# trappmartin/DeepStructuredMixtures

Hardware: AMD Instinct MI355X
Metric: fit!+predict wall-clock, DSMGP N=100k D=8 (lower is better)
Workload: dtype f64

## Files before the change

deepstructuredmixtures_amd/csrc/dsmgp_hip.cpp:

```cpp
#include "../../include/dsmgp_hip.h"
#ifdef DSMGP_DIAG
#include "../../include/dsmgp_hip_diag.h"
#endif
#include "kernels.hpp"
#include "kernels_fused.hpp"

#include <algorithm>
#include <atomic>
#include <cmath>
#include <cstdio>
#include <cstdlib>
#include <cstring>
#include <string>
#include <thread>
#include <array>
#include <chrono>
#include <dlfcn.h>
#include <limits>
#include <vector>

using namespace dsmgp;

namespace {

std::string g_create_error;

struct HyperHost {
    int kind = -1;
    std::vector<double> loghyp;
};

struct LeafHost {
    int n = 0, npad = 0, nb = 0, kid = 0;
    double mean = 0.0;
    int64_t obs_off = 0;
    int op = DSMGP_SHARE_FULL, src = -1;
    int64_t prefix = 0;
    int owner = -1;
    int kb = 0;
    size_t f_off = 0, dinv_off = 0, vec_off = 0, xg_off = 0;
    int nt = 0, ntpad = 0;
    size_t vt_off = 0, xt_off = 0, pv_off = 0;
    int64_t route_off = 0;
};

template <class T>
struct DevBuf {
    T* p = nullptr;
    size_t count = 0;
    size_t cap = 0;

    DevBuf() = default;
    DevBuf(const DevBuf&) = delete;
    DevBuf& operator=(const DevBuf&) = delete;
    DevBuf(DevBuf&& o) noexcept : p(o.p), count(o.count), cap(o.cap) {
        o.p = nullptr;
        o.count = o.cap = 0;
    }
    DevBuf& operator=(DevBuf&& o) noexcept {
        if (this != &o) {
            release();
            std::swap(p, o.p);
            std::swap(count, o.count);
            std::swap(cap, o.cap);
        }
        return *this;
    }
    ~DevBuf() { release(); }

    int grow(dsmgp_ctx* c, size_t need, size_t want);
    int grow(dsmgp_ctx* c, size_t need) { return grow(c, need, std::max<size_t>(1, need + need / 8)); }
    int alloc(dsmgp_ctx* c, size_t n) { return grow(c, n, n); }
    void clear() { count = 0; }
    void release() {
        if (p) (void)hipFree(p);
        p = nullptr;
        count = cap = 0;
    }
    void drop(bool keep) { keep ? clear() : release(); }
};

struct HostLog {
    const char* what;
    std::chrono::steady_clock::time_point t0;
    explicit HostLog(const char* w) : what(w), t0(std::chrono::steady_clock::now()) {}
    void lap(const char* next) {
        done();
        what = next;
        t0 = std::chrono::steady_clock::now();
    }
    void done() {
        static const bool on = std::getenv("DSMGP_HOSTLOG") != nullptr;
        if (on && what)
            std::fprintf(stderr, "hostlog %-28s %.4f s\n", what,
                         std::chrono::duration<double>(std::chrono::steady_clock::now() - t0).count());
        what = nullptr;
    }
    ~HostLog() { done(); }
};

enum { STEP_CLASSIC = 0, STEP_FUSED = 1 };
constexpr int MAX_LANES = 4;
#ifndef DSMGP_FUSED_SHALLOW
#define DSMGP_FUSED_SHALLOW 4
#endif
constexpr int FUSED_SHALLOW_STEPS = DSMGP_FUSED_SHALLOW;
constexpr int FUSED_SHALLOW_MIN_LEAVES = 32;
#ifndef DSMGP_STREAM_FLAGS
#define DSMGP_STREAM_FLAGS hipStreamDefault
#endif
#ifndef DSMGP_LANES_AUTO_MIN
#define DSMGP_LANES_AUTO_MIN 8
#endif
constexpr int LANES_AUTO_MIN_LEAVES = DSMGP_LANES_AUTO_MIN;
#ifndef DSMGP_TAIL_SPLIT_DEFAULT
#define DSMGP_TAIL_SPLIT_DEFAULT 4
#endif
#ifndef DSMGP_TAIL_ROUNDS_DEFAULT
#define DSMGP_TAIL_ROUNDS_DEFAULT 1
#endif
#ifndef DSMGP_TAIL_SPLIT_LANES
#define DSMGP_TAIL_SPLIT_LANES 1
// ... 193 lines not shown
        const size_t T = tiles.size();
        size_t slab = 0;
        if ((int)T < ncu) {
            tail_begin = upd.size();
            emit(tiles, 0, T, choose_split((int)T, K, ncu), slab);
        } else {
            const size_t r = T % (size_t)ncu;
            size_t ntail = r + (T < (size_t)(2 * ncu) ? (size_t)tail_rounds * ncu : 0);
            if (ntail > T) ntail = T;
            int S = std::min(tail_split, std::max(1, K / 256));
            if (r > 0 && r * 4 < (size_t)ncu) S = std::max(S, (int)std::min<size_t>((size_t)ncu / r, 16));
            S = std::min(S, std::max(1, K / 256));
            if (S <= 1 || r == 0) ntail = 0;
            emit(tiles, 0, T - ntail, 1, slab);
            tail_begin = upd.size();
            if (ntail) emit(tiles, T - ntail, T, S, slab);
        }
        max_slabs = std::max(max_slabs, slab);
    }
    int ragged_rounds = 2, ragged_div = 4;
    void add_step_ragged(const std::vector<TileTask>& tiles, int Kavg, int kblocks) {
        const size_t T = tiles.size();
        if (kblocks < 8) {
            add_step(tiles, Kavg);
            return;
        }
        size_t slab = 0;
        size_t cut = 0;
        int maxb;
        if (T < (size_t)((ragged_rounds + 2) * ncu)) {
            long W = 0;
            for (const TileTask& u : tiles) W += (u.k1 - u.k0) / TB;
            maxb = (int)std::min<long>(kblocks, std::max<long>(2, W / (long)(2 * ncu * 3)));
        } else {
            cut = T - (size_t)(ragged_rounds * ncu);
            emit(tiles, 0, cut, 1, slab);
            maxb = std::max(1, kblocks / ragged_div);
        }
        auto pieces = [&](const TileTask& u) { return std::max(1, ((u.k1 - u.k0) / TB + maxb - 1) / maxb); };
        for (size_t i = cut; i < T;) {
            const int S = pieces(tiles[i]);
            size_t j = i + 1;
            while (j < T && pieces(tiles[j]) == S) ++j;
            emit(tiles, i, j, S, slab);
            i = j;
        }
        max_slabs = std::max(max_slabs, slab);
    }
    void bind(double* workspace) {
        for (size_t i = 0; i < upd.size(); ++i)
            if (upd_slab[i] >= 0) upd[i].C = workspace + (size_t)upd_slab[i] * TB * TB;
        for (size_t i = 0; i < red.size(); ++i) red[i].slabs = workspace + (size_t)red_slab[i] * TB * TB;
    }
};

struct SweepLane {
    UpdateSplitter U;
    std::vector<TileTask> trsm;
    std::vector<int> upd_at, red_at, trsm_at;
    void mark(int k) {
        upd_at[(size_t)k] = (int)U.upd.size();
        red_at[(size_t)k] = (int)U.red.size();
        trsm_at[(size_t)k] = (int)trsm.size();
    }
};

}

struct dsmgp_ctx {
    int device = 0;
    hipStream_t stream = nullptr;
    std::string err;
    int profile = 0;
    bool alt_names = false;

    int64_t N = 0;
    int D = 0;
    DevBuf<double> dX, dy;

    int L = 0;
    std::vector<LeafHost> leaves;
    std::vector<int64_t> obs_ptr, obs_idx;
    DevBuf<int64_t> d_obs_ptr, d_obs_idx;
    bool plan_ready = false;

    std::vector<HyperHost> hyper;
    DevBuf<KParam> d_kp;
    DevBuf<double> d_l2;

    double* arenaF = nullptr;
    double* arenaDinv = nullptr;
    double* arenaVec = nullptr;
    double* arenaXg = nullptr;
    DevBuf<int> d_info;
    DevBuf<int> d_owner;
    DevBuf<double> d_mll;
    DevBuf<LeafDev> d_leaves;
    std::vector<LeafDev> h_leaves;
    size_t bytes_needed = 0;

    DevBuf<GramTask> gram;
    bool fuse_gram = true;
    bool fuse_steps = true;
    bool diag_in_update = true;
    std::vector<char> fused_step[2];
    int lanes_opt = 0;
    int nlanes = 1;
    hipStream_t lane_stream[MAX_LANES] = {};
    hipEvent_t ev_fork = nullptr, ev_join[MAX_LANES] = {};
    std::vector<char> leaf_lane;
    StepLists phase[MAX_LANES][2];
    std::vector<char> leaf_group;
    char* pool_base = nullptr;
    size_t pool_cap = 0, pool_top = 0, pool_mark_plan = 0;
    double* slabF[MAX_LANES] = {};
    StepLists phaseJ[MAX_LANES][2];
    double* slabJ[MAX_LANES] = {};
    double alg_flops_joint = 0.0;
    bool joint = true;
    bool joint_ready = false;
    bool vt_valid = false;
    bool last_fit_joint = false;
    int ncu = 256;
    bool xcd_order = true;
    int tail_split = DSMGP_TAIL_SPLIT_DEFAULT, tail_rounds = DSMGP_TAIL_ROUNDS_DEFAULT;
    int tail_split_lanes = DSMGP_TAIL_SPLIT_LANES, tail_rounds_lanes = DSMGP_TAIL_ROUNDS_LANES;
    int ragged_rounds = 2, ragged_div = 4;
    std::vector<int> fwd_off, bwd_off;
    DevBuf<SolveTask> fwd, bwd;
    int solve_steps = 0;
    bool fitted = false;
    bool use_graph = false;
    hipGraphExec_t fit_graph[2] = {nullptr, nullptr};
    int graph_launches[2][2] = {{0, 0}, {0, 0}};
    bool alpha_valid = false;
    bool dinv_complete = false;
    DevBuf<DiagTask> dinvc_prefix;
    DevBuf<DiagTask> dinvc_fwd;
    DevBuf<DiagTask> dinvc_all;

    DevBuf<double> dXt;
    int64_t n_t = 0;
    DevBuf<int64_t> d_route_ptr, d_route_idx;
    std::vector<int64_t> route_ptr;
    double* arenaVt = nullptr;
    size_t arenaVt_count = 0;
    size_t cap_Xt = 0, cap_PV = 0;
    char* stage = nullptr;
    size_t stage_cap = 0, stage_top = 0;
    DevBuf<SweepSeg> psegs;
    double* arenaXt = nullptr;
    double* arenaPV = nullptr;
    size_t acc_off = 0, acc_count = 0;
    DevBuf<PredTask> ptasks_slow;
    DevBuf<GramTask> pgram;
    DevBuf<GramTask> pgram0;
    DevBuf<PredTask> ptasks;
    SweepLists psweep;
    double* arenaCov = nullptr;
    size_t cap_Cov = 0;
    DevBuf<PredCovTask> pcov;
    double* arenaB = nullptr;
    size_t cap_B = 0;
    DevBuf<PredBetaTask> pgbeta;
    DevBuf<PredGradTask> pgtasks;
    DevBuf<PredGradFinTask> pgfin;
    DevBuf<double> d_pgpart;
    DevBuf<double> d_pgout;
    bool test_ready = false;
    bool predicted = false;
    int64_t route_total = 0;

    DevBuf<int64_t> d_row_ptr;
    DevBuf<int32_t> d_row_ent;
    DevBuf<int32_t> d_ent_leaf;
    DevBuf<double> d_agg_part;
    DevBuf<double> d_agg_coef;
    DevBuf<int32_t> d_agg_group;
    DevBuf<double> d_agg_out;
    int agg_family = -1, agg_G = 0, agg_W = 0;
    bool agg_partial_ready = false, agg_done = false;
    bool agg_total = false;

    bool grad_ready = false;
    std::vector<char> grad_active;
    double* arenaX = nullptr;
    size_t arenaX_count = 0;
    DevBuf<TransTask> gtrans;
    SweepLists ginv;
    DevBuf<FrobTask> gfrob;
    std::vector<int> gfrob_leaf;
    DevBuf<GradTask> gdot;
    size_t gdot_prod0 = 0;
    size_t gdot_mat0 = 0;
    std::vector<int> gdot_leaf;
    DevBuf<ArdLinTask> gardlin;
    std::vector<int> gardlin_leaf;
    bool ard_true_gradient = false;
    int gstride = 2;
    std::vector<int> grad_src;
    DevBuf<double> d_gpart;
    size_t gpart_count = 0;
    bool xinv_all = false;
    bool grad_lists_all = false;
    bool grad_all_owners = false;
    std::vector<size_t> gxoff;
    bool loo_ready = false;
    DevBuf<RowNormTask> lrow;
    DevBuf<LooTask> lleaf;
    DevBuf<double> d_loo;
    bool lg_ready = false;
    std::vector<int> lg_kinds;
// ... 211 lines not shown
    }
    S.upd_off[(size_t)nv] = bu;
    S.red_off[(size_t)nv] = br;
    S.trsm_off[(size_t)nv] = bt;
    return 0;
}

void drop_graphs(dsmgp_ctx* c) {
    for (auto& g : c->fit_graph)
        if (g) {
            (void)hipGraphExecDestroy(g);
            g = nullptr;
        }
}

void free_grad_lists(dsmgp_ctx* c) {
    c->gtrans.clear();
    c->ginv.clear();
    c->gfrob.clear();
    c->gdot.clear();
    c->gardlin.clear();
    c->grad_ready = false;
}

void free_grad(dsmgp_ctx* c) {
    c->ginv.release(c);
    arena_put(c, c->arenaX);
    c->gtrans.release();
    c->gfrob.release();
    c->gdot.release();
    c->gardlin.release();
    c->d_gpart.release();
    c->grad_ready = false;
    c->xinv_all = false;
    c->loo_ready = false;
    c->lrow.release();
    c->lleaf.release();
    c->d_loo.release();
    c->lg_ready = false;
    arena_put(c, c->arenaH);
    c->d_lgvec.release();
    c->lgvec.release();
    c->lginv.release();
    c->lghvec.release();
    c->lgdot.release();
    c->lgardlin.release();
    c->d_lgpart.release();
}

void free_tree(dsmgp_ctx* c) {
    c->rtree = RouteTree{};
    c->rt_kind.release();
    c->rt_first.release();
    c->rt_nchild.release();
    c->rt_sdim.release();
    c->rt_leaf.release();
    c->rt_thr.release();
    c->rtree_ready = false;
    c->rtree_nodes = 0;
    c->rtree_max_leaf = -1;
}

void free_test(dsmgp_ctx* c, bool keep = false);
void free_plan(dsmgp_ctx* c) {
    drop_graphs(c);
    if (c->pool_base) {
        free_test(c);
        c->pool_top = 0;
        c->pool_mark_plan = 0;
    }
    arena_put(c, c->arenaF);
    arena_put(c, c->arenaDinv);
    arena_put(c, c->arenaVec);
    arena_put(c, c->arenaXg);
    c->d_info.release();
    c->d_owner.release();
    c->d_mll.release();
    c->d_leaves.release();
    c->gram.release();
    for (auto& lane : c->phase)
        for (auto& ph : lane) ph.drop(false);
    for (auto& sl : c->slabF) arena_put(c, sl);
    c->fwd.release();
    c->bwd.release();
    c->dinvc_prefix.release();
    c->dinvc_fwd.release();
    c->dinvc_all.release();
    free_grad(c);
    c->plan_ready = false;
    c->phase_ready = false;
    c->fitted = false;
}

void free_test(dsmgp_ctx* c, bool keep) {
    drop_graphs(c);
    if (c->pool_base) {
        free_grad(c);
        c->pool_top = c->pool_mark_plan;
        keep = false;
    }
    c->dXt.drop(keep);
    c->d_route_ptr.drop(keep);
    c->d_route_idx.drop(keep);
    c->d_row_ptr.drop(keep);
    c->d_row_ent.drop(keep);
    c->d_ent_leaf.drop(keep);
    c->d_agg_part.drop(keep);
    c->d_agg_coef.drop(keep);
    c->d_agg_group.drop(keep);
    c->d_agg_out.drop(keep);
    c->agg_partial_ready = c->agg_done = c->agg_total = false;
    if (!keep) {
        arena_put(c, c->arenaVt);
        c->arenaVt_count = 0;
        arena_put(c, c->arenaXt);
        arena_put(c, c->arenaPV);
        c->cap_Xt = c->cap_PV = 0;
    }
    c->pgram.drop(keep);
    c->pgram0.drop(keep);
    c->ptasks.drop(keep);
    c->ptasks_slow.drop(keep);
    c->psweep.drop(c, keep);
    c->psegs.drop(keep);
    arena_put(c, c->arenaCov);
    c->cap_Cov = 0;
    c->pcov.drop(keep);
    arena_put(c, c->arenaB);
    c->cap_B = 0;
    c->pgbeta.drop(keep);
    c->pgtasks.drop(keep);
    c->pgfin.drop(keep);
    c->d_pgpart.drop(keep);
    c->d_pgout.drop(keep);
    for (auto& lane : c->phaseJ)
        for (auto& ph : lane) ph.drop(keep);
    for (auto& sl : c->slabJ) arena_put(c, sl);
    c->joint_ready = false;
    c->vt_valid = false;
    c->test_ready = false;
    c->predicted = false;
}

inline int round_up(int x, int m) { return (x + m - 1) / m * m; }
inline int tile_mrows(int valid) {
    const int m = round_up(std::max(0, std::min(TB, valid)), 16);
    return m >= TB ? 0 : std::max(16, m);
}

struct KindInfo {
    const char* name;
    bool ard;
    bool iso_matern;
    bool matern;
    bool linear;
    double nh_num;
    bool per_dim_grad;
    bool contraction;
    bool set_checked;
};
constexpr KindInfo KINDS[] = {
    {"IsoSE",          false, false, false, false, -0.5,  false,  true,  false},
    {"ArdSE",          true,  false, false, false, -0.5,  true,   false, false},
    {"IsoLinear",      false, false, false, true,  -0.5,  false,  false, false},
    {"ArdLinear",      true,  false, false, true,  1.0,   false,  false, false},
    {"ArdSEProduct",   true,  false, false, false, -0.5,  true,   true,  true},
// ... 108 lines not shown

bool gram_fused(const dsmgp_ctx* c) { return c->fuse_gram && c->D <= GRAM_FUSE_MAX_D; }

void push_fused8_tasks(std::vector<FusedTask8>& out, std::vector<RowBlock>& blocks, const LeafDev& d, const LeafHost& lf, int k) {
    for (size_t b0 = 0; b0 < blocks.size(); b0 += 8) {
        FusedTask8 f{};
        f.B = d.F + (size_t)k * TB;
        f.Dinv = d.Dinv + (size_t)k * TB * TB;
        f.gxb = d.Xg + (size_t)k * TB;
        f.ldb = f.gldb = lf.npad;
        f.gnb = std::max(0, std::min(TB, lf.n - k * TB));
        f.k1 = k * TB;
        f.kid = lf.kid;
        f.nblk = (int)std::min<size_t>(8, blocks.size() - b0);
        for (int q = 0; q < f.nblk; ++q) {
            f.rb[q] = blocks[b0 + q];
            if (f.rb[q].wi != nullptr) f.zk = d.z + (size_t)k * TB;
        }
        out.push_back(f);
    }
    blocks.clear();
}

int build_factor_steps(dsmgp_ctx* c, int lane, bool with_test, StepLists (&phase)[2], double*& slab_ws, double& alg_flops,
                       double& alg_flops_fused, bool slab_outside_pool = false) {
    const int L = c->L;
    alg_flops = 0.0;
    const bool fused = gram_fused(c);
    UpdateSplitter split[2] = {make_splitter(c, c->nlanes), make_splitter(c, c->nlanes)};
    for (int ph = 0; ph < 2; ++ph) {
        StepLists& S = phase[ph];
        UpdateSplitter& U = split[ph];
        auto in_phase = [&](const LeafHost& lf) {
            const size_t l = (size_t)(&lf - c->leaves.data());
            return c->leaf_group[l] == ph && c->leaf_lane[l] == lane;
        };
        int nsteps = 0;
        for (int l = 0; l < L; ++l) {
            const LeafHost& lf = c->leaves[l];
            if (!in_phase(lf)) continue;
            if (lf.owner == l || (with_test && lf.nt > 0)) nsteps = std::max(nsteps, lf.nb);
        }
        S.nsteps = nsteps;
        std::vector<TileTask> trsm;
        std::vector<DiagTask> diag;
        std::vector<FusedTask8> ftile8;
        std::vector<RowBlock> blocks8;
        std::vector<DiagFusedTask> fdiag;
        std::vector<DiagFinishTask> dfin;
        S.dpos.assign(nsteps, 0);
        S.dfin_off.assign(nsteps + 1, 0);
        S.upd_off.assign(nsteps + 1, 0);
        S.red_off.assign(nsteps + 1, 0);
        S.trsm_off.assign(nsteps + 1, 0);
        S.diag_off.assign(nsteps + 1, 0);
        S.fdiag_off.assign(nsteps + 1, 0);
        S.ftile8_off.assign(nsteps + 1, 0);
        S.step_tiles.assign(nsteps, 0);
        S.pad.assign(nsteps, 0);
        S.mode.assign(nsteps, STEP_CLASSIC);
        for (int k = 0; k < nsteps; ++k) {
            S.upd_off[k] = (int)U.upd.size();
            S.red_off[k] = (int)U.red.size();
            S.trsm_off[k] = (int)trsm.size();
            S.diag_off[k] = (int)diag.size();
            S.fdiag_off[k] = (int)fdiag.size();
            S.ftile8_off[k] = (int)ftile8.size();
            S.dfin_off[k] = (int)dfin.size();
            const int mode = k < (int)c->fused_step[ph].size() ? c->fused_step[ph][k] : STEP_CLASSIC;
            S.mode[k] = (char)mode;
            const bool fstep = mode != STEP_CLASSIC;
            std::vector<TileTask> tiles;
            auto classic_at = [&](int q) {
                return q >= 0 && q < nsteps && (q >= (int)c->fused_step[ph].size() || c->fused_step[ph][q] == STEP_CLASSIC);
            };
            const bool finish_here = c->diag_in_update && gram_fused(c) && !fstep && k >= 2 && classic_at(k - 1);
            const bool ahead = c->diag_in_update && gram_fused(c) && !fstep && k >= 1 && classic_at(k + 1);
            size_t nsym = 0;
            for (int l = 0; l < L; ++l) {
                const LeafHost& lf = c->leaves[l];
                if (lf.nb <= k || !in_phase(lf)) continue;
                const LeafDev& d = c->h_leaves[l];
                const int ld = lf.npad;
                if (lf.owner == l) {
                    const int i_first = (k < lf.kb) ? lf.kb : k;
                    const bool own_diag = (k >= lf.kb);
                    const bool fin = finish_here && own_diag;
                    for (int i = i_first; i < lf.nb; ++i) {
                        if (fstep) {
                            if (i == k) continue;
                            const int rows = std::max(0, std::min(TB, lf.n - i * TB));
                            for (int r = 0; r < rows; r += 16) {
                                RowBlock b{};
                                b.A = d.F + (size_t)i * TB + r;
                                b.C = d.F + (size_t)i * TB + r + (size_t)k * TB * ld;
                                b.gx = d.Xg + (size_t)i * TB + r;
                                b.lda = b.ldc = b.glda = ld;
                                b.nvalid = std::min(16, rows - r);
                                if (ph != 1) b.wi = d.w + (size_t)i * TB + r;
                                blocks8.push_back(b);
                            }
                            continue;
                        }
                        if (k > 0 && !(i == k && fin)) {
                            TileTask u{};
                            u.A = d.F + (size_t)i * TB;
                            u.B = d.F + (size_t)k * TB;
                            u.C = d.F + (size_t)i * TB + (size_t)k * TB * ld;
                            u.lda = u.ldb = u.ldc = ld;
                            u.k0 = 0;
                            u.k1 = k * TB;
                            u.update = 1;
                            u.mrows = tile_mrows(lf.n - i * TB);
                            u.sym = (i == k) ? 1 : 0;
                            nsym += (size_t)u.sym;
                            if (fused) {
                                u.gram = 1 | (i == k ? 2 : 0) | 4;
                                u.kid = lf.kid;
                                u.gxa = d.Xg + (size_t)i * TB;
                                u.gxb = d.Xg + (size_t)k * TB;
                                u.glda = u.gldb = ld;
                                u.gna = std::max(0, std::min(TB, lf.n - i * TB));
                                u.gnb = std::max(0, std::min(TB, lf.n - k * TB));
                            }
                            tiles.push_back(u);
                        }
                        if (i == k + 1 && ahead && k + 1 >= lf.kb) {
                            TileTask u{};
                            u.A = u.B = d.F + (size_t)i * TB;
                            u.C = d.F + (size_t)i * TB + (size_t)i * TB * ld;
                            u.lda = u.ldb = u.ldc = ld;
                            u.k0 = 0;
                            u.k1 = k * TB;
                            u.update = 1;
                            u.mrows = tile_mrows(lf.n - i * TB);
                            u.sym = 1;
                            nsym += 1;
                            u.gram = 1 | 2 | 4;
                            u.kid = lf.kid;
                            u.gxa = u.gxb = d.Xg + (size_t)i * TB;
                            u.glda = u.gldb = ld;
                            u.gna = u.gnb = std::max(0, std::min(TB, lf.n - i * TB));
                            tiles.push_back(u);
                        }
                        if (i > k) {
                            TileTask s{};
                            s.A = d.F + (size_t)i * TB + (size_t)k * TB * ld;
                            s.B = d.Dinv + (size_t)k * TB * TB;
                            s.C = const_cast<double*>(s.A);
                            s.lda = ld;
                            s.ldb = TB;
                            s.ldc = ld;
                            s.k0 = 0;
                            s.k1 = TB;
                            s.update = 0;
                            s.mrows = tile_mrows(lf.n - i * TB);
                            if (ph != 1) {
                                s.zk = d.z + (size_t)k * TB;
                                s.wi = d.w + (size_t)i * TB;
                            }
                            trsm.push_back(s);
                        }
                    }
                    if (own_diag) {
                        DiagTask g{};
                        g.T = d.F + (size_t)k * TB + (size_t)k * TB * ld;
                        g.Dinv = d.Dinv + (size_t)k * TB * TB;
                        if (ph != 1) {
                            g.wk = d.w + (size_t)k * TB;
                            g.zk = d.z + (size_t)k * TB;
                        }
                        g.info = d.info;
                        g.ld = ld;
                        g.nvalid = std::max(0, std::min(TB, lf.n - k * TB));
                        g.row0 = k * TB;
                        if (fstep) {
                            DiagFusedTask fg{};
                            fg.d = g;
                            fg.A = d.F + (size_t)k * TB;
                            fg.gx = d.Xg + (size_t)k * TB;
                            fg.k1 = k * TB;
                            fg.glda = ld;
                            fg.kid = lf.kid;
                            fdiag.push_back(fg);
                        } else if (fin) {
                            DiagFinishTask ft{};
                            ft.d = g;
                            ft.A = d.F + (size_t)k * TB + (size_t)(k - 1) * TB * ld;
                            dfin.push_back(ft);
                        } else {
                            diag.push_back(g);
                        }
                    }
                }
                if (with_test && lf.nt > 0) {
                    for (int ti = 0; ti < lf.ntpad / TB; ++ti) {
                        double* tile = d.Vt + (size_t)ti * TB + (size_t)k * TB * lf.ntpad;
                        if (fstep) {
                            const int rows = std::max(0, std::min(TB, lf.nt - ti * TB));
                            for (int r = 0; r < rows; r += 16) {
                                RowBlock b{};
                                b.A = d.Vt + (size_t)ti * TB + r;
                                b.C = tile + r;
                                b.gx = d.Xtg + (size_t)ti * TB + r;
                                b.lda = b.ldc = b.glda = lf.ntpad;
                                b.nvalid = std::min(16, rows - r);
                                if (d.zfused) {
                                    b.wi = d.macc + (size_t)ti * TB + r;
                                    b.sq = d.sacc + (size_t)ti * TB + r;
                                }
                                blocks8.push_back(b);
                            }
                            continue;
                        }
                        if (k > 0) {
                            TileTask u{};
                            u.A = d.Vt + (size_t)ti * TB;
                            u.B = d.F + (size_t)k * TB;
                            u.C = tile;
                            u.lda = lf.ntpad;
                            u.ldb = ld;
                            u.ldc = lf.ntpad;
                            u.k0 = 0;
                            u.k1 = k * TB;
                            u.update = 1;
                            u.mrows = tile_mrows(lf.nt - ti * TB);
                            if (fused) {
                                u.gram = 1;
                                u.kid = lf.kid;
                                u.gxa = d.Xtg + (size_t)ti * TB;
                                u.gxb = d.Xg + (size_t)k * TB;
                                u.glda = lf.ntpad;
                                u.gldb = ld;
                                u.gna = std::max(0, std::min(TB, lf.nt - ti * TB));
                                u.gnb = std::max(0, std::min(TB, lf.n - k * TB));
                            }
                            tiles.push_back(u);
                        }
                        TileTask s{};
                        s.A = tile;
                        s.B = d.Dinv + (size_t)k * TB * TB;
                        s.C = tile;
                        s.lda = lf.ntpad;
                        s.ldb = TB;
                        s.ldc = lf.ntpad;
                        s.k0 = 0;
                        s.k1 = TB;
                        s.update = 0;
                        s.mrows = tile_mrows(lf.nt - ti * TB);
                        if (d.zfused) {
                            s.zk = d.z + (size_t)k * TB;
// ... 153 lines not shown
        HIPCHK(c, hipMemcpy(c->d_owner.p, owner.data(), (size_t)L * sizeof(int), hipMemcpyHostToDevice));
    }
    if (int rc = c->d_mll.alloc(c, L)) return rc;
    if (int rc = c->d_leaves.alloc(c, L)) return rc;

    c->h_leaves.assign(L, LeafDev{});
    for (int l = 0; l < L; ++l) {
        const LeafHost& lf = c->leaves[l];
        LeafDev& d = c->h_leaves[l];
        d.F = c->arenaF + lf.f_off;
        d.Dinv = c->arenaDinv + lf.dinv_off;
        d.Xg = c->arenaXg + lf.xg_off;
        d.yc = c->arenaVec + lf.vec_off;
        d.w = d.yc + lf.npad;
        d.z = d.w + lf.npad;
        d.alpha = d.z + lf.npad;
        d.info = c->d_info.p + lf.owner;
        d.mean = lf.mean;
        d.n = lf.n;
        d.npad = lf.npad;
        d.nb = lf.nb;
        d.kid = lf.kid;
    }
    HIPCHK(c, hipMemcpy(c->d_leaves.p, c->h_leaves.data(), L * sizeof(LeafDev), hipMemcpyHostToDevice));

    {
        int maxpad = 0;
        for (auto& lf : c->leaves) maxpad = std::max(maxpad, lf.npad);
        for (int l0 = 0; l0 < L; l0 += 32768) {
            const int cnt = std::min(32768, L - l0);
            dim3 grid((maxpad + 255) / 256, cnt);
            gather_leaf_kernel<<<grid, 256, 0, c->stream>>>(c->d_leaves.p, c->d_obs_ptr.p, c->d_obs_idx.p, c->dX.p, c->dy.p,
                                                            c->N, c->D, l0);
        }
        HIPCHK(c, hipGetLastError());
    }
    std::vector<ZeroRowsTask> zr;
    if (gram_fused(c)) {
        for (int l = 0; l < L; ++l) {
            const LeafHost& lf = c->leaves[l];
            const int last = lf.n - (lf.nb - 1) * TB;
            if (lf.owner != l || lf.nb < 2 || last >= TB) continue;
            ZeroRowsTask z{};
            z.p = c->h_leaves[l].F + (size_t)(lf.nb - 1) * TB;
            z.ld = lf.npad;
            z.r0 = (std::max(0, last) + 15) / 16 * 16;
            z.ncols = (lf.nb - 1) * TB;
            if (z.r0 < TB) zr.push_back(z);
        }
    }
    std::vector<ZeroUpperTask> zu;
    int maxnb = 1;
    for (int l = 0; l < L; ++l) {
        const LeafHost& lf = c->leaves[l];
        if (lf.owner != l) continue;
        zu.push_back(ZeroUpperTask{c->h_leaves[l].F, lf.npad, lf.nb});
        maxnb = std::max(maxnb, lf.nb);
    }
    {
        DevBuf<ZeroRowsTask> zrows;
        DevBuf<ZeroUpperTask> zupper;
        if (int rc = dev_upload(c, zrows, zr)) return rc;
        if (int rc = dev_upload(c, zupper, zu)) return rc;
        if (!zr.empty()) zero_pad_rows_kernel<<<(int)zr.size(), 256, 0, c->stream>>>(zrows.p);
        for (size_t b0 = 0; b0 < zu.size(); b0 += 32768) {
            const size_t cnt = std::min<size_t>(32768, zu.size() - b0);
            zero_upper_blocks_kernel<<<dim3((unsigned)cnt, (unsigned)std::min(maxnb, 64)), 256, 0, c->stream>>>(zupper.p + b0);
        }
        const hipError_t e1 = hipGetLastError(), e2 = hipStreamSynchronize(c->stream);
        HIPCHK(c, e1);
        HIPCHK(c, e2);
    }

    c->leaf_group.assign(L, 0);
    for (int l = 0; l < L; ++l)
        if (c->leaves[l].op == DSMGP_SHARE_PREFIX) c->leaf_group[l] = 1;
    {
        std::vector<int> unit(L);
        std::vector<double> cost(L, 0.0);
        for (int l = 0; l < L; ++l) {
            const LeafHost& lf = c->leaves[l];
            unit[l] = lf.op == DSMGP_SHARE_FULL ? l : lf.src;
            const double n = (double)lf.n;
            cost[unit[l]] += lf.op == DSMGP_SHARE_COPY ? n * n : n * n * n;
        }
        int nunits = 0;
        for (int l = 0; l < L; ++l) nunits += unit[l] == l ? 1 : 0;
        c->nlanes = c->lanes_opt > 0 ? c->lanes_opt : (nunits >= LANES_AUTO_MIN_LEAVES ? 2 : 1);
        c->nlanes = std::max(1, std::min(c->nlanes, nunits));
        c->leaf_lane.assign(L, 0);
        if (c->nlanes > 1) {
            std::vector<int> order;
            for (int l = 0; l < L; ++l)
                if (unit[l] == l) order.push_back(l);
            std::stable_sort(order.begin(), order.end(), [&](int a, int b) { return cost[a] > cost[b]; });
            double load[MAX_LANES] = {};
            std::vector<char> of_unit(L, 0);
            for (int u : order) {
                int lane = 0;
                for (int q = 1; q < c->nlanes; ++q)
                    if (load[q] < load[lane]) lane = q;
                of_unit[u] = (char)lane;
                load[lane] += cost[u];
            }
            for (int l = 0; l < L; ++l) c->leaf_lane[l] = of_unit[unit[l]];
        }
    }
    for (int ph = 0; ph < 2; ++ph) {
        int ns = 0;
        for (int l = 0; l < L; ++l)
            if (c->leaf_group[l] == ph) ns = std::max(ns, c->leaves[l].nb);
        c->fused_step[ph].assign(ns, STEP_CLASSIC);
        if (!gram_fused(c)) continue;
        for (int k = 0; k < ns; ++k) {
            int nd = 0;
            for (int l = 0; l < L; ++l) {
                const LeafHost& lf = c->leaves[l];
                if (c->leaf_group[l] == ph && lf.owner == l && lf.nb > k && k >= lf.kb) ++nd;
            }
            if (c->fuse_steps && (nd > c->ncu || (k <= FUSED_SHALLOW_STEPS && nd >= FUSED_SHALLOW_MIN_LEAVES))) c->fused_step[ph][k] = STEP_FUSED;
        }
    }
    std::vector<GramTask> gram;
    const bool fused = gram_fused(c);
    for (int l = 0; l < L; ++l) {
        const LeafHost& lf = c->leaves[l];
        if (lf.owner != l) continue;
        {
            const std::vector<char>& fs = c->fused_step[(int)c->leaf_group[l]];
            if (fused && !fs.empty() && fs[0] != STEP_CLASSIC) continue;
        }
        const LeafDev& d = c->h_leaves[l];
        for (int j = 0; j < (fused ? 1 : lf.nb); ++j)
            for (int i = (fused ? std::max(j, lf.kb) : j); i < lf.nb; ++i) {
                GramTask g{};
                g.xa = d.Xg + (size_t)i * TB;
                g.xb = d.Xg + (size_t)j * TB;
                g.out = d.F + (size_t)i * TB + (size_t)j * TB * lf.npad;
                g.lda = g.ldb = g.ldo = lf.npad;
                g.na = std::max(0, std::min(TB, lf.n - i * TB));
                g.nb = std::max(0, std::min(TB, lf.n - j * TB));
                g.sym = 1;
                g.diag = (i == j);
                g.kid = lf.kid;
                gram.push_back(g);
            }
    }
    if (int rc = dev_upload(c, c->gram, gram)) return rc;

    {
        auto fused_in = [&](int ph, int k) { return k < (int)c->fused_step[ph].size() && c->fused_step[ph][k] == STEP_FUSED; };
        auto block_task = [&](int l, int k) {
            const LeafHost& lf = c->leaves[l];
            const LeafDev& d = c->h_leaves[l];
            DiagTask g{};
            g.T = d.F + (size_t)k * TB + (size_t)k * TB * lf.npad;
            g.Dinv = d.Dinv + (size_t)k * TB * TB;
            g.info = d.info;
            g.ld = lf.npad;
            g.nvalid = std::max(0, std::min(TB, lf.n - k * TB));
            g.row0 = k * TB;
            return g;
        };
        std::vector<DiagTask> pre, fw;
        std::vector<char> done(L, 0);
        for (int l = 0; l < L; ++l) {
            const LeafHost& lf = c->leaves[l];
            if (lf.op == DSMGP_SHARE_PREFIX)
                for (int k = 0; k < lf.kb; ++k)
                    if (fused_in(0, k)) pre.push_back(block_task(l, k));
            if (lf.op == DSMGP_SHARE_FULL) continue;
            const int o = lf.owner;
            if (done[o]) continue;
            done[o] = 1;
            const LeafHost& lo = c->leaves[o];
            const int pho = (int)c->leaf_group[o];
            for (int k = lo.kb; k < lo.nb; ++k)
                if (fused_in(pho, k)) fw.push_back(block_task(o, k));
        }
        if (int rc = dev_upload(c, c->dinvc_prefix, pre)) return rc;
        if (int rc = dev_upload(c, c->dinvc_fwd, fw)) return rc;
        std::vector<DiagTask> all;
        for (int l = 0; l < L; ++l) {
            const LeafHost& lf = c->leaves[l];
            if (lf.owner != l) continue;
            for (int k = lf.kb; k < lf.nb; ++k)
                if (fused_in((int)c->leaf_group[l], k)) all.push_back(block_task(l, k));
        }
        if (int rc = dev_upload(c, c->dinvc_all, all)) return rc;
    }
    c->phase_ready = false;

    {
        int nsteps = 0;
        for (auto& lf : c->leaves) nsteps = std::max(nsteps, lf.nb);
        c->solve_steps = nsteps;
        std::vector<SolveTask> fwd, bwd;
        c->fwd_off.assign(nsteps + 1, 0);
        c->bwd_off.assign(nsteps + 1, 0);
        for (int k = 0; k < nsteps; ++k) {
            c->fwd_off[k] = (int)fwd.size();
            for (int l = 0; l < L; ++l) {
                const LeafHost& lf = c->leaves[l];
                if (lf.nb <= k) continue;
                if (lf.owner == l && lf.op == DSMGP_SHARE_FULL) continue;
                const LeafDev& d = c->h_leaves[l];
                for (int i = k; i < lf.nb; ++i) {
                    SolveTask s{};
                    s.Dk = d.Dinv + (size_t)k * TB * TB;
                    s.vk = d.w + (size_t)k * TB;
                    s.ldt = lf.npad;
                    if (i == k) {
                        s.self = 1;
                        s.out_k = d.z + (size_t)k * TB;
                    } else {
                        s.T = d.F + (size_t)i * TB + (size_t)k * TB * lf.npad;
                        s.vi = d.w + (size_t)i * TB;
                    }
                    fwd.push_back(s);
                }
            }
        }
        c->fwd_off[nsteps] = (int)fwd.size();
        for (int s_ = 0; s_ < nsteps; ++s_) {
            c->bwd_off[s_] = (int)bwd.size();
            for (int l = 0; l < L; ++l) {
                const LeafHost& lf = c->leaves[l];
                const LeafDev& d = c->h_leaves[l];
                if (s_ == 0) {
                    SolveTask s{};
                    s.self = 1;
                    s.Dk = d.Dinv + (size_t)(lf.nb - 1) * TB * TB;
                    s.vk = d.w + (size_t)(lf.nb - 1) * TB;
                    s.out_k = d.alpha + (size_t)(lf.nb - 1) * TB;
                    s.ldt = lf.npad;
                    bwd.push_back(s);
                    continue;
                }
                const int kb = lf.nb - s_;
                if (kb < 1) continue;
                for (int j = 0; j < kb; ++j) {
                    SolveTask s{};
                    s.T = d.F + (size_t)kb * TB + (size_t)j * TB * lf.npad;
                    s.ldt = lf.npad;
                    s.vk = d.alpha + (size_t)kb * TB;
                    s.vi = d.w + (size_t)j * TB;
                    if (j == kb - 1) {
                        s.Dk = d.Dinv + (size_t)j * TB * TB;
                        s.out_k = d.alpha + (size_t)j * TB;
                    }
                    bwd.push_back(s);
                }
            }
        }
        c->bwd_off[nsteps] = (int)bwd.size();
        if (int rc = dev_upload(c, c->fwd, fwd)) return rc;
        if (int rc = dev_upload(c, c->bwd, bwd)) return rc;
    }
    HIPCHK(c, hipStreamSynchronize(c->stream));
    c->plan_ready = true;
    c->pool_mark_plan = c->pool_top;
    return 0;
}

int ensure_phase(dsmgp_ctx* c) {
    if (c->phase_ready) return 0;
    HostLog hl("ensure_phase: factor steps");
    c->alg_flops_update = c->alg_flops_fused = 0.0;
    for (int lane = 0; lane < c->nlanes; ++lane) {
        double fu = 0.0, ff = 0.0;
        if (int rc = build_factor_steps(c, lane, false, c->phase[lane], c->slabF[lane], fu, ff, true)) return rc;
        c->alg_flops_update += fu;
        c->alg_flops_fused += ff;
    }
    HIPCHK(c, hipStreamSynchronize(c->stream));
    c->phase_ready = true;
    return 0;
}

int ensure_joint(dsmgp_ctx* c) {
    if (c->joint_ready) return 0;
    HostLog hl("ensure_joint: joint factor steps");
    c->alg_flops_joint = c->alg_flops_fused_joint = 0.0;
    for (int lane = 0; lane < c->nlanes; ++lane) {
        double fu = 0.0, ff = 0.0;
        if (int rc = build_factor_steps(c, lane, true, c->phaseJ[lane], c->slabJ[lane], fu, ff)) return rc;
        c->alg_flops_joint += fu;
        c->alg_flops_fused_joint += ff;
    }
    HIPCHK(c, hipStreamSynchronize(c->stream));
    c->joint_ready = true;
    return 0;
}

void launch_tiles(dsmgp_ctx* c, const TileTask* tasks, int n, int role = 0 , bool pad = false,
                  int dpos = 0, const DiagFinishTask* dfin = nullptr, int ndfin = 0, hipStream_t st = nullptr) {
    const int g = n + ndfin;
    if (!st) st = c->stream;
    if (pad) {
        if (role == 1) tile_trsm_kernel<true><<<n, 256, 0, st>>>(tasks);
        else if (c->profile == 0 || c->alt_names) tile_gemm_kernel_v2<false, 2, true><<<g, 256, 0, st>>>(tasks, nullptr, c->d_kp.p, c->D, dpos, dfin, ndfin);
        else tile_gemm_kernel_v2<false, 0, true><<<g, 256, 0, st>>>(tasks, nullptr, c->d_kp.p, c->D, dpos, dfin, ndfin);
        return;
    }
    if (role == 1) tile_trsm_kernel<false><<<n, 256, 0, st>>>(tasks);
    else if (c->profile == 0 || c->alt_names) tile_gemm_kernel_v2<false, 2><<<g, 256, 0, st>>>(tasks, nullptr, c->d_kp.p, c->D, dpos, dfin, ndfin);
// ... 114 lines not shown
        pt.end(st);
        const int nr = S.red_off[k + 1] - S.red_off[k];
        if (nr > 0) {
            pt.begin(13, st);
            tile_reduce_kernel<<<nr * REDUCE_WGS, 256, 0, st>>>(S.red.p + S.red_off[k]);
            pt.end(st);
        }
        if (count_launches) c->n_update_launches++;
    }
    const int nd = S.diag_off[k + 1] - S.diag_off[k];
    if (nd > 0) {
        pt.begin(2, st);
        chol_diag_packed_kernel<<<nd, 256, DIAGP_LDS_BYTES, st>>>(S.diag.p + S.diag_off[k]);
        pt.note(k, nd, 0);
        pt.end(st);
    }
    const int ns = S.trsm_off[k + 1] - S.trsm_off[k];
    if (ns > 0) {
        pt.begin(3, st);
        launch_tiles(c, S.trsm.p + S.trsm_off[k], ns, 1, S.pad[k] != 0, 0, nullptr, 0, st);
        pt.note(k, ns, 0);
        pt.end(st);
    }
}

int fork_lanes(dsmgp_ctx* c, int nl) {
    if (nl > 1) {
        HIPCHK(c, hipEventRecord(c->ev_fork, c->stream));
        for (int lane = 1; lane < nl; ++lane) HIPCHK(c, hipStreamWaitEvent(c->lane_stream[lane], c->ev_fork, 0));
    }
    return 0;
}
int join_lanes(dsmgp_ctx* c, int nl) {
    for (int lane = 1; lane < nl; ++lane) {
        HIPCHK(c, hipEventRecord(c->ev_join[lane], c->lane_stream[lane]));
        HIPCHK(c, hipStreamWaitEvent(c->stream, c->ev_join[lane], 0));
    }
    return 0;
}

int run_lanes(dsmgp_ctx* c, StepLists (*lists)[2], int ph, PhaseTimer& pt, bool count_launches) {
    int nsteps = 0;
    for (int lane = 0; lane < c->nlanes; ++lane) nsteps = std::max(nsteps, lists[lane][ph].nsteps);
    if (nsteps == 0) return 0;
    if (int rc = fork_lanes(c, c->nlanes)) return rc;
    for (int k = 0; k < nsteps; ++k)
        for (int lane = 0; lane < c->nlanes; ++lane) run_step(c, lists[lane][ph], k, pt, c->lane_stream[lane], count_launches);
    HIPCHK(c, hipGetLastError());
    return join_lanes(c, c->nlanes);
}

int ensure_dinv(dsmgp_ctx* c) {
    if (c->dinv_complete) return 0;
    if (c->dinvc_all.count)
        dinv_complete_kernel<<<(int)c->dinvc_all.count, 256, DIAGP_LDS_BYTES, c->stream>>>(c->dinvc_all.p);
    HIPCHK(c, hipGetLastError());
    c->dinv_complete = true;
    return 0;
}

int ensure_alpha(dsmgp_ctx* c) {
    if (c->alpha_valid) return 0;
    if (int rc = ensure_dinv(c)) return rc;
    EventPair ev;
    HIPCHK(c, ev.init());
    HIPCHK(c, hipEventRecord(ev.a, c->stream));
    int maxpad = 0;
    for (auto& lf : c->leaves) maxpad = std::max(maxpad, lf.npad);
    copy_z_kernel<<<dim3((maxpad + 255) / 256, c->L), 256, 0, c->stream>>>(c->d_leaves.p);
    for (int s = 0; s < c->solve_steps; ++s) {
        const int n = c->bwd_off[s + 1] - c->bwd_off[s];
        if (n > 0) solve_bwd_kernel<<<n, 256, 0, c->stream>>>(c->bwd.p + c->bwd_off[s]);
    }
    HIPCHK(c, hipGetLastError());
    HIPCHK(c, hipEventRecord(ev.b, c->stream));
    HIPCHK(c, hipStreamSynchronize(c->stream));
    float ms = 0.f;
    HIPCHK(c, hipEventElapsedTime(&ms, ev.a, ev.b));
    c->timings[14] = ms * 1e-3;
    c->alpha_valid = true;
    return 0;
}

}

extern "C" {

int dsmgp_create(int32_t device_id, dsmgp_ctx** out) {
    if (!out) return fail(nullptr, DSMGP_E_ARG, "out is NULL");
    *out = nullptr;
    int ndev = 0;
    if (hipGetDeviceCount(&ndev) != hipSuccess || ndev == 0)
        return fail(nullptr, DSMGP_E_NODEVICE, "no HIP device visible: the GP-expert path has no CPU fallback");
    if (device_id < 0 || device_id >= ndev) return fail(nullptr, DSMGP_E_ARG, "device id out of range");
    dsmgp_ctx* c = new dsmgp_ctx();
    c->device = device_id;
    if (hipSetDevice(device_id) != hipSuccess || hipStreamCreateWithFlags(&c->stream, DSMGP_STREAM_FLAGS) != hipSuccess) {
        delete c;
        return fail(nullptr, DSMGP_E_HIP, "cannot initialise device");
    }
    c->lane_stream[0] = c->stream;
    bool lanes_ok = hipEventCreateWithFlags(&c->ev_fork, hipEventDisableTiming) == hipSuccess;
    for (int lane = 1; lane < MAX_LANES && lanes_ok; ++lane)
        lanes_ok = hipStreamCreateWithFlags(&c->lane_stream[lane], DSMGP_STREAM_FLAGS) == hipSuccess &&
                   hipEventCreateWithFlags(&c->ev_join[lane], hipEventDisableTiming) == hipSuccess;
    if (!lanes_ok) {
        (void)hipStreamDestroy(c->stream);
        delete c;
        return fail(nullptr, DSMGP_E_HIP, "cannot create the lanes' streams");
    }
    (void)hipFuncSetAttribute(reinterpret_cast<const void*>(chol_diag_packed_kernel),
                              hipFuncAttributeMaxDynamicSharedMemorySize, DIAGP_LDS_BYTES);
    (void)hipFuncSetAttribute(reinterpret_cast<const void*>(dinv_complete_kernel),
                              hipFuncAttributeMaxDynamicSharedMemorySize, DIAGP_LDS_BYTES);
    {
        hipDeviceProp_t prop;
        if (hipGetDeviceProperties(&prop, device_id) == hipSuccess && prop.multiProcessorCount > 0)
            c->ncu = prop.multiProcessorCount;
    }
#ifdef DSMGP_DIAG
    if (const char* s = std::getenv("DSMGP_XCD")) c->xcd_order = std::atoi(s) != 0;
    if (const char* s = std::getenv("DSMGP_TAIL_SPLIT")) c->tail_split = c->tail_split_lanes = std::max(1, std::atoi(s));
    if (const char* s = std::getenv("DSMGP_TAIL_ROUNDS")) c->tail_rounds = c->tail_rounds_lanes = std::max(0, std::atoi(s));
    if (const char* s = std::getenv("DSMGP_RAGGED_ROUNDS")) c->ragged_rounds = std::max(1, std::atoi(s));
    if (const char* s = std::getenv("DSMGP_RAGGED_DIV")) c->ragged_div = std::max(1, std::atoi(s));
#endif
    const char* p = std::getenv("DSMGP_PROFILE");
    c->profile = p ? std::atoi(p) * 2 : 0;
    *out = c;
    return 0;
}

int dsmgp_destroy(dsmgp_ctx* c) {
    if (!c) return DSMGP_E_ARG;
    (void)hipSetDevice(c->device);
    free_plan(c);
    free_test(c);
    if (c->pool_base) (void)hipFree(c->pool_base);
    c->pool_base = nullptr;
    (void)dsmgp_comm_destroy(c);
    drop_graphs(c);
    if (c->side) {
        (void)hipStreamSynchronize(c->side);
        (void)hipStreamDestroy(c->side);
    }
    if (c->stage) (void)hipHostFree(c->stage);
    c->stage = nullptr;
    for (hipEvent_t e : c->event_pool) (void)hipEventDestroy(e);
    if (c->ev_fork) (void)hipEventDestroy(c->ev_fork);
    for (int lane = 1; lane < MAX_LANES; ++lane) {
        if (c->ev_join[lane]) (void)hipEventDestroy(c->ev_join[lane]);
        if (c->lane_stream[lane]) (void)hipStreamDestroy(c->lane_stream[lane]);
    }
    if (c->stream) (void)hipStreamDestroy(c->stream);
    delete c;
    return 0;
}

const char* dsmgp_last_error(dsmgp_ctx* c) { return c ? c->err.c_str() : g_create_error.c_str(); }

int dsmgp_device_name(dsmgp_ctx* c, char* buf, int32_t len) {
    if (!c || !buf || len <= 0) return DSMGP_E_ARG;
    hipDeviceProp_t prop;
    HIPCHK(c, hipGetDeviceProperties(&prop, c->device));
    std::snprintf(buf, len, "%s (%s, %d CUs)", prop.name, prop.gcnArchName, prop.multiProcessorCount);
    return 0;
}

int dsmgp_set_joint(dsmgp_ctx* c, int32_t on) {
    if (!c) return DSMGP_E_ARG;
    c->joint = on != 0;
    return 0;
}

int dsmgp_set_option(dsmgp_ctx* c, int32_t option, int32_t value) {
    if (!c) return DSMGP_E_ARG;
    if (option == DSMGP_OPT_ARD_LENGTHSCALE_GRADIENT) {
        if ((value != 0) != c->ard_true_gradient) {
            HIPCHK(c, hipSetDevice(c->device));
            free_grad(c);
        }
        c->ard_true_gradient = value != 0;
        return 0;
    }
    if (option == DSMGP_OPT_FUSED_GRAM) {
        if ((value != 0) != c->fuse_gram) {
            HIPCHK(c, hipSetDevice(c->device));
            free_plan(c);
            free_test(c);
        }
        c->fuse_gram = value != 0;
        return 0;
    }
    if (option == DSMGP_OPT_FUSED_STEPS) {
        if ((value != 0) != c->fuse_steps) {
            HIPCHK(c, hipSetDevice(c->device));
            free_plan(c);
            free_test(c);
        }
        c->fuse_steps = value != 0;
        return 0;
    }
    if (option == DSMGP_OPT_FIT_GRAPH) {
        if (value == 0) drop_graphs(c);
        c->use_graph = value != 0;
        return 0;
    }
    if (option == DSMGP_OPT_LANES) {
        if (value < 0 || value > MAX_LANES) return fail(c, DSMGP_E_ARG, "set_option: lanes must be 0 (automatic) or 1 .. 4");
        if (value != c->lanes_opt) {
            HIPCHK(c, hipSetDevice(c->device));
            free_plan(c);
            free_test(c);
        }
        c->lanes_opt = value;
        return 0;
    }
    if (option == DSMGP_OPT_DIAG_IN_UPDATE) {
        if ((value != 0) != c->diag_in_update) {
            HIPCHK(c, hipSetDevice(c->device));
            free_plan(c);
            free_test(c);
        }
        c->diag_in_update = value != 0;
        return 0;
    }
    return fail(c, DSMGP_E_ARG, "set_option: unknown option");
}

int dsmgp_set_profile(dsmgp_ctx* c, int32_t on) {
    if (!c) return DSMGP_E_ARG;
    c->alt_names = on == 3;
    c->profile = on < 0 ? 0 : (on == 3 ? 1 : (on > 2 ? 2 : on));
    return 0;
}

int dsmgp_set_train(dsmgp_ctx* c, const double* X, const double* y, int64_t N, int32_t D) {
    if (!c) return DSMGP_E_ARG;
    if (!X || !y || N <= 0 || D <= 0) return fail(c, DSMGP_E_ARG, "set_train: bad arguments");
    HIPCHK(c, hipSetDevice(c->device));
    free_plan(c);
    free_test(c);
    free_tree(c);
    c->dX.release();
    c->dy.release();
    c->N = N;
    c->D = D;
    if (int rc = c->dX.alloc(c, (size_t)N * D)) return rc;
    if (int rc = c->dy.alloc(c, (size_t)N)) return rc;
    HIPCHK(c, hipMemcpy(c->dX.p, X, (size_t)N * D * sizeof(double), hipMemcpyHostToDevice));
    HIPCHK(c, hipMemcpy(c->dy.p, y, (size_t)N * sizeof(double), hipMemcpyHostToDevice));
    c->L = 0;
    c->leaves.clear();
    return 0;
}

int dsmgp_set_leaves(dsmgp_ctx* c, int32_t L, const int64_t* obs_ptr, const int64_t* obs_idx,
                     const int32_t* kernel_id, const double* mean) {
    if (!c) return DSMGP_E_ARG;
    if (!c->dX.p) return fail(c, DSMGP_E_STATE, "set_leaves before set_train");
    if (L <= 0 || !obs_ptr || !obs_idx || !kernel_id || !mean) return fail(c, DSMGP_E_ARG, "set_leaves: bad arguments");
    HIPCHK(c, hipSetDevice(c->device));
    free_plan(c);
    free_test(c);
    free_tree(c);
    if (obs_ptr[0] != 0) return fail(c, DSMGP_E_ARG, "obs_ptr[0] must be 0");
    c->leaves.assign(L, LeafHost{});
    c->grad_active.clear();
    for (int l = 0; l < L; ++l) {
        const int64_t a = obs_ptr[l], b = obs_ptr[l + 1];
        if (b <= a) return fail(c, DSMGP_E_ARG, "leaf " + std::to_string(l) + " has no observations");
        if (b - a > (int64_t)1 << 20) return fail(c, DSMGP_E_ARG, "leaf too large");
        for (int64_t i = a; i < b; ++i) {
            if (obs_idx[i] < 0 || obs_idx[i] >= c->N) return fail(c, DSMGP_E_ARG, "observation index out of range");
            if (i > a && obs_idx[i] <= obs_idx[i - 1]) return fail(c, DSMGP_E_ARG, "obs lists must be strictly ascending");
        }
        if (kernel_id[l] < 0 || kernel_id[l] >= DSMGP_MAX_KERNEL_IDS) return fail(c, DSMGP_E_ARG, "kernel id out of range");
        LeafHost& lf = c->leaves[l];
        lf.n = (int)(b - a);
        lf.npad = round_up(lf.n, TB);
        lf.nb = lf.npad / TB;
        lf.kid = kernel_id[l];
        lf.mean = mean[l];
        lf.obs_off = a;
    }
    c->L = L;
    c->obs_ptr.assign(obs_ptr, obs_ptr + L + 1);
    c->obs_idx.assign(obs_idx, obs_idx + obs_ptr[L]);
    c->d_obs_ptr.release();
    c->d_obs_idx.release();
    if (int rc = c->d_obs_ptr.alloc(c, (size_t)L + 1)) return rc;
    if (int rc = c->d_obs_idx.grow(c, c->obs_idx.size(), std::max<size_t>(1, c->obs_idx.size()))) return rc;
    HIPCHK(c, hipMemcpy(c->d_obs_ptr.p, obs_ptr, (L + 1) * sizeof(int64_t), hipMemcpyHostToDevice));
    HIPCHK(c, hipMemcpy(c->d_obs_idx.p, obs_idx, c->obs_idx.size() * sizeof(int64_t), hipMemcpyHostToDevice));
    return 0;
}

int dsmgp_set_sharing(dsmgp_ctx* c, const int32_t* op, const int32_t* src, const int64_t* prefix_len) {
    if (!c) return DSMGP_E_ARG;
    if (c->L == 0) return fail(c, DSMGP_E_STATE, "set_sharing before set_leaves");
    const int L = c->L;
    struct Share { int op; int src; int64_t prefix; };
    std::vector<Share> sh(L, Share{DSMGP_SHARE_FULL, -1, 0});
    for (int l = 0; l < L; ++l) {
        const LeafHost& lf = c->leaves[l];
        const int o = op ? op[l] : DSMGP_SHARE_FULL;
        if (o == DSMGP_SHARE_FULL) continue;
        if (!src || src[l] < 0 || src[l] >= L || src[l] == l) return fail(c, DSMGP_E_ARG, "sharing: bad source leaf");
        const LeafHost& s = c->leaves[src[l]];
        const int so = op[src[l]];
        if (so != DSMGP_SHARE_FULL) return fail(c, DSMGP_E_ARG, "sharing: source leaf must be factorised in full");
        if (s.kid != lf.kid) return fail(c, DSMGP_E_ARG, "sharing: kernel ids differ");
        const int64_t* a = c->obs_idx.data() + lf.obs_off;
        const int64_t* b = c->obs_idx.data() + s.obs_off;
        if (o == DSMGP_SHARE_COPY) {
            if (s.n != lf.n || std::memcmp(a, b, sizeof(int64_t) * lf.n) != 0)
                return fail(c, DSMGP_E_ARG, "sharing: COPY needs identical observation lists");
            sh[l] = Share{o, src[l], 0};
        } else if (o == DSMGP_SHARE_PREFIX) {
            if (!prefix_len || prefix_len[l] != s.n || s.n >= lf.n || std::memcmp(a, b, sizeof(int64_t) * s.n) != 0)
                return fail(c, DSMGP_E_ARG, "sharing: PREFIX needs the source's list as a strict prefix");
            sh[l] = Share{o, src[l], prefix_len[l]};
        } else {
            return fail(c, DSMGP_E_ARG, "sharing: unknown op");
        }
    }
    HIPCHK(c, hipSetDevice(c->device));
    free_plan(c);
    free_test(c);
    for (int l = 0; l < L; ++l) {
        c->leaves[l].op = sh[l].op;
        c->leaves[l].src = sh[l].src;
        c->leaves[l].prefix = sh[l].prefix;
    }
    return 0;
}

int dsmgp_set_hyper(dsmgp_ctx* c, int32_t kernel_id, int32_t kind, const double* loghyp, int32_t n) {
    if (!c) return DSMGP_E_ARG;
    if (kernel_id < 0 || kernel_id >= DSMGP_MAX_KERNEL_IDS || !loghyp || n < 3) return fail(c, DSMGP_E_ARG, "set_hyper: bad arguments");
    if (kind < 0 || kind > DSMGP_KIND_ARD_MATERN52) return fail(c, DSMGP_E_ARG, "set_hyper: unknown kernel kind");
    const KindInfo& ki = KINDS[kind];
    if (ki.set_checked && ki.ard && c->D > 0 && n != c->D + 2)
        return fail(c, DSMGP_E_ARG, std::string("set_hyper: ") + ki.name + " needs one lengthscale per input dimension");
    if (ki.set_checked && !ki.ard && n != 3)
        return fail(c, DSMGP_E_ARG, std::string("set_hyper: ") + ki.name + " takes [logl, logs, logNoise]");
    for (int i = 0; i < n; ++i)
        if (!std::isfinite(loghyp[i])) return fail(c, DSMGP_E_ARG, "set_hyper: non-finite hyper-parameter");
    if ((int)c->hyper.size() <= kernel_id) c->hyper.resize(kernel_id + 1);
    const bool had_matern = any_matern(c);
    if (c->hyper[kernel_id].kind != kind) free_grad(c);
    c->hyper[kernel_id].kind = kind;
    c->hyper[kernel_id].loghyp.assign(loghyp, loghyp + n);
    if (any_matern(c) != had_matern) drop_graphs(c);
    c->fitted = false;
    c->predicted = false;
    c->vt_valid = false;
    return 0;
}

int dsmgp_fit(dsmgp_ctx* c, double* mll_out, int32_t* info_out, double* seconds) {
    if (!c) return DSMGP_E_ARG;
    if (c->L == 0) return fail(c, DSMGP_E_STATE, "fit before set_leaves");
    HIPCHK(c, hipSetDevice(c->device));
    if (int rc = check_hyper(c)) return rc;
    if (!c->plan_ready)
        if (int rc = build_plan(c)) return rc;
    if (int rc = upload_hyper(c)) return rc;
    const bool joint = c->joint && c->test_ready;
    if (joint) {
        if (int rc = ensure_joint(c)) return rc;
    } else if (int rc = ensure_phase(c)) {
        return rc;
    }
    const int L = c->L;
    for (int i = 0; i < 6; ++i) c->timings[i] = 0.0;
    c->timings[11] = 0.0;
    c->timings[13] = 0.0;
    c->timings[14] = 0.0;
    c->timings[18] = c->timings[19] = c->timings[20] = 0.0;
    c->n_update_launches = 0;
    c->n_fused_launches = 0;
    PhaseTimer pt(c);
    EventPair ev;
    HIPCHK(c, ev.init());
    const hipEvent_t t0 = ev.a, t1 = ev.b;
    HIPCHK(c, hipEventRecord(t0, c->stream));

    StepLists (*phases)[2] = joint ? c->phaseJ : c->phase;
    auto enqueue = [&]() -> int {
        HIPCHK(c, hipMemsetAsync(c->d_info.p, 0, L * sizeof(int), c->stream));
        if (joint && c->acc_count) HIPCHK(c, hipMemsetAsync(c->arenaPV + c->acc_off, 0, c->acc_count * sizeof(double), c->stream));
        {
            const DevBuf<GramTask>& tg = (joint && gram_fused(c)) ? c->pgram0 : c->pgram;
            pt.begin(0);
            if (c->gram.count) gram_tile_kernel<<<2 * (int)c->gram.count, 256, 0, c->stream>>>(c->gram.p, c->d_kp.p, c->D);
            if (joint && tg.count) gram_tile_kernel<<<2 * (int)tg.count, 256, 0, c->stream>>>(tg.p, c->d_kp.p, c->D);
            pt.end();
        }
        {
            int maxpad = 0;
            for (auto& lf : c->leaves) maxpad = std::max(maxpad, lf.npad);
            copy_vec_kernel<<<dim3((maxpad + 255) / 256, L), 256, 0, c->stream>>>(c->d_leaves.p);
        }
        if (int rc = run_lanes(c, phases, 0, pt, true)) return rc;
        bool any_prefix = false;
        for (int l = 0; l < L; ++l) {
            const LeafHost& lf = c->leaves[l];
            if (lf.op != DSMGP_SHARE_PREFIX) continue;
            any_prefix = true;
            const LeafDev& d = c->h_leaves[l];
            const LeafDev& s = c->h_leaves[lf.src];
            const size_t rows = (size_t)lf.kb * TB;
            HIPCHK(c, hipMemcpy2DAsync(d.F, (size_t)d.npad * sizeof(double), s.F, (size_t)s.npad * sizeof(double),
                                       rows * sizeof(double), rows, hipMemcpyDeviceToDevice, c->stream));
            HIPCHK(c, hipMemcpyAsync(d.Dinv, s.Dinv, rows * TB * sizeof(double), hipMemcpyDeviceToDevice, c->stream));
        }
        if (any_prefix) {
            if (c->dinvc_prefix.count)
                dinv_complete_kernel<<<(int)c->dinvc_prefix.count, 256, DIAGP_LDS_BYTES, c->stream>>>(c->dinvc_prefix.p);
            if (int rc = run_lanes(c, phases, 1, pt, true)) return rc;
        }
        {
            pt.begin(4);
            if (c->dinvc_fwd.count)
                dinv_complete_kernel<<<(int)c->dinvc_fwd.count, 256, DIAGP_LDS_BYTES, c->stream>>>(c->dinvc_fwd.p);
            for (int k = 0; k < c->solve_steps; ++k) {
                const int n = c->fwd_off[k + 1] - c->fwd_off[k];
                if (n > 0) solve_fwd_kernel<<<n, 256, 0, c->stream>>>(c->fwd.p + c->fwd_off[k]);
            }
            pt.end();
        }
        pt.begin(5);
        mll_kernel<<<L, 256, 0, c->stream>>>(c->d_leaves.p, c->d_mll.p);
        pt.end();
        return 0;
    };
    c->vt_valid = false;
    c->alpha_valid = false;
    c->xinv_all = false;
    const int gk = joint ? 1 : 0;
    if (c->use_graph && c->profile == 0) {
        if (!c->fit_graph[gk]) {
            hipGraph_t g = nullptr;
            HIPCHK(c, hipStreamBeginCapture(c->stream, hipStreamCaptureModeThreadLocal));
            const int rc = enqueue();
            const hipError_t ce = hipStreamEndCapture(c->stream, &g);
            if (rc != 0 || ce != hipSuccess || !g) {
                if (g) (void)hipGraphDestroy(g);
                (void)hipGetLastError();
                c->use_graph = false;
                if (rc != 0) return rc;
            } else {
                const hipError_t ie = hipGraphInstantiate(&c->fit_graph[gk], g, nullptr, nullptr, 0);
                (void)hipGraphDestroy(g);
                if (ie != hipSuccess) {
                    c->fit_graph[gk] = nullptr;
                    (void)hipGetLastError();
                    c->use_graph = false;
                }
                c->graph_launches[gk][0] = c->n_update_launches;
                c->graph_launches[gk][1] = c->n_fused_launches;
            }
        }
        if (c->fit_graph[gk]) {
            HIPCHK(c, hipGraphLaunch(c->fit_graph[gk], c->stream));
            c->n_update_launches = c->graph_launches[gk][0];
            c->n_fused_launches = c->graph_launches[gk][1];
        } else if (int rc = enqueue()) {
            return rc;
        }
    } else {
        if (int rc = enqueue()) return rc;
    }
    HIPCHK(c, hipGetLastError());
    HIPCHK(c, hipEventRecord(t1, c->stream));
    HIPCHK(c, hipStreamSynchronize(c->stream));
    float ms = 0.f;
    HIPCHK(c, hipEventElapsedTime(&ms, t0, t1));
    pt.collect(t0);
    c->timings[11] = ms * 1e-3;
    if (seconds) *seconds = ms * 1e-3;
    if (mll_out) HIPCHK(c, hipMemcpy(mll_out, c->d_mll.p, L * sizeof(double), hipMemcpyDeviceToHost));
    if (info_out) {
        std::vector<int> owner_info(L);
        HIPCHK(c, hipMemcpy(owner_info.data(), c->d_info.p, L * sizeof(int), hipMemcpyDeviceToHost));
        for (int l = 0; l < L; ++l) info_out[l] = owner_info[c->leaves[l].owner];
    }
    c->fitted = true;
    c->predicted = false;
    c->vt_valid = joint;
    c->last_fit_joint = joint;
    c->dinv_complete = c->dinvc_all.count == 0;
    return 0;
}

}

namespace {
int register_test(dsmgp_ctx* c, HostLog& hl) {
    const int L = c->L;
    const int64_t n_t = c->n_t, total = c->route_total;
    const int64_t* rp = c->route_ptr.data();
    hl.lap("set_test: sizes");
    size_t vTot = 0, xTot = 0;
    size_t accTot = 0;
    for (int l = 0; l < L; ++l) accTot += (size_t)round_up((int)(rp[l + 1] - rp[l]), TB);
    const size_t pTot = 2 * (size_t)total + 2 * accTot + 2 * TB;
    for (int l = 0; l < L; ++l) {
        LeafHost& lf = c->leaves[l];
        lf.nt = (int)(rp[l + 1] - rp[l]);
        lf.ntpad = round_up(lf.nt, TB);
        lf.route_off = rp[l];
        lf.vt_off = vTot;
        vTot += (size_t)lf.ntpad * lf.npad;
        lf.xt_off = xTot;
        xTot += (size_t)lf.ntpad * c->D;
        lf.pv_off = (size_t)rp[l];
    }
    size_t freeB = 0, totalB = 0;
    HIPCHK(c, hipMemGetInfo(&freeB, &totalB));
    const size_t need = (vTot + xTot + pTot) * sizeof(double) + (size_t)n_t * c->D * sizeof(double);
    if (!c->pool_base) freeB += (c->arenaVt_count + c->cap_Xt + c->cap_PV) * sizeof(double);
    if (!c->pool_base && need + (size_t(1) << 30) > freeB)
        return fail(c, DSMGP_E_NOMEM, "test set needs " + std::to_string(need >> 20) + " MiB, device has " +
                                          std::to_string(freeB >> 20) + " MiB free");
    hl.lap("set_test: arenas");
    auto arena_fit = [&](double*& p, size_t& cap, size_t need_) -> int {
        if (c->pool_base) return arena_get(c, p, need_);
        if (p && cap >= need_ && cap <= 2 * need_ + (size_t(1) << 20)) return 0;
        arena_put(c, p);
        cap = 0;
        const size_t want = need_ + need_ / 8;
        if (int rc = arena_get(c, p, want)) return rc;
        cap = want;
        return 0;
    };
    if (int rc = arena_fit(c->arenaVt, c->arenaVt_count, vTot)) return rc;
    if (int rc = arena_fit(c->arenaXt, c->cap_Xt, xTot)) return rc;
    if (int rc = arena_fit(c->arenaPV, c->cap_PV, pTot)) return rc;
    int maxpad = 0;
    size_t accOff = 0;
    c->acc_off = 2 * (size_t)total;
    c->acc_count = 2 * accTot;
    for (int l = 0; l < L; ++l) {
        const LeafHost& lf = c->leaves[l];
        LeafDev& d = c->h_leaves[l];
        d.Vt = c->arenaVt + lf.vt_off;
        d.Xtg = c->arenaXt + lf.xt_off;
        d.mu = c->arenaPV + lf.pv_off;
        d.var = c->arenaPV + (size_t)total + lf.pv_off;
        d.macc = c->arenaPV + 2 * (size_t)total + accOff;
        d.sacc = d.macc + accTot;
        d.zfused = (lf.owner == l && lf.op == DSMGP_SHARE_FULL) ? 1 : 0;
        accOff += (size_t)lf.ntpad;
        d.nt = lf.nt;
        d.ntpad = lf.ntpad;
        maxpad = std::max(maxpad, lf.ntpad);
    }
    if (int rc = stage_upload(c, c->d_leaves.p, c->h_leaves.data(), (size_t)L * sizeof(LeafDev))) return rc;
    if (maxpad > 0) {
        for (int l0 = 0; l0 < L; l0 += 32768) {
            const int cnt = std::min(32768, L - l0);
            gather_test_kernel<<<dim3((maxpad + 255) / 256, cnt), 256, 0, c->stream>>>(
                c->d_leaves.p, c->d_route_ptr.p, c->d_route_idx.p, c->dXt.p, n_t, c->D, l0);
        }
        HIPCHK(c, hipGetLastError());
    }
    hl.lap("set_test: task lists (host)");
    auto fused_at = [&](int l, int k) {
        const std::vector<char>& fs = c->fused_step[(int)c->leaf_group[l]];
        return gram_fused(c) && k < (int)fs.size() && fs[(size_t)k] == STEP_FUSED;
    };
    std::vector<GramTask> pg, pg0;
    std::vector<PredTask> ptk, ptk_slow;
    int nsteps = 0;
    for (int l = 0; l < L; ++l) {
        const LeafHost& lf = c->leaves[l];
        if (lf.nt == 0) continue;
        nsteps = std::max(nsteps, lf.nb);
        const LeafDev& d = c->h_leaves[l];
        for (int ti = 0; ti < lf.ntpad / TB; ++ti) {
            ptk.push_back(PredTask{l, ti * TB});
            if (!d.zfused) ptk_slow.push_back(PredTask{l, ti * TB});
            for (int j = 0; j < lf.nb; ++j) {
                if (fused_at(l, j)) continue;
                if (j > 0 && gram_fused(c)) continue;
                GramTask g{};
                g.xa = d.Xtg + (size_t)ti * TB;
                g.xb = d.Xg + (size_t)j * TB;
                g.out = d.Vt + (size_t)ti * TB + (size_t)j * TB * lf.ntpad;
                g.lda = lf.ntpad;
                g.ldb = lf.npad;
                g.ldo = lf.ntpad;
                g.na = std::max(0, std::min(TB, lf.nt - ti * TB));
                g.nb = std::max(0, std::min(TB, lf.n - j * TB));
                g.sym = 0;
                g.diag = 0;
                g.kid = lf.kid;
                pg.push_back(g);
                if (j == 0) pg0.push_back(g);
            }
        }
    }
    const int nl = c->nlanes, nv = nl * nsteps;
    std::vector<SweepLane> lanes = sweep_lanes(c, nl, nsteps);
    std::vector<int>& f8_off = c->psweep.f8_off;
    f8_off.assign((size_t)nv + 1, 0);
    std::vector<SweepSeg> segs;
    std::vector<std::vector<int>> classic((size_t)nv);
    {
        std::vector<int> cnt8((size_t)nv, 0);
        for (int l = 0; l < L; ++l) {
            const LeafHost& lf = c->leaves[l];
            if (lf.nt == 0) continue;
            const int nt8 = ((lf.nt + 15) / 16 + 7) / 8;
            const size_t v0 = (size_t)c->leaf_lane[l] * (size_t)nsteps;
            for (int k = 0; k < lf.nb; ++k) {
                if (fused_at(l, k)) cnt8[v0 + (size_t)k] += nt8;
                else classic[v0 + (size_t)k].push_back(l);
            }
        }
        for (int v = 0; v < nv; ++v) f8_off[(size_t)v + 1] = f8_off[(size_t)v] + cnt8[(size_t)v];
        std::vector<int> cursor((size_t)nv, 0);
        segs.reserve((size_t)L * 4);
        for (int l = 0; l < L; ++l) {
            const LeafHost& lf = c->leaves[l];
            if (lf.nt == 0) continue;
            const int nt8 = ((lf.nt + 15) / 16 + 7) / 8;
            const size_t v0 = (size_t)c->leaf_lane[l] * (size_t)nsteps;
            for (int k = 0; k < lf.nb; ++k)
                if (fused_at(l, k)) {
                    SweepSeg sg{};
                    sg.leaf = l;
                    sg.k = k;
                    sg.src0 = cursor[v0 + (size_t)k];
                    sg.begin = f8_off[v0 + (size_t)k];
// ... 961 lines not shown
        c->grad_all_owners = false;
        if (rc) return rc;
    }
    return 0;
}
int xinv_fill(dsmgp_ctx* c) {
    if (c->xinv_all) return 0;
    if (c->gtrans.count) transpose_tile_kernel<<<(int)c->gtrans.count * 16, 256, 0, c->stream>>>(c->gtrans.p);
    return run_sweep(c, c->ginv, nullptr);
}

int build_loo_plan(dsmgp_ctx* c) {
    const int L = c->L;
    std::vector<size_t> poff(L, 0);
    size_t pTot = 0;
    for (int l = 0; l < L; ++l) {
        const LeafHost& lf = c->leaves[l];
        if (lf.owner != l) continue;
        poff[l] = pTot;
        pTot += (size_t)lf.npad * ((lf.n + ROWNORM_COLS - 1) / ROWNORM_COLS);
    }
    const size_t nobs = (size_t)c->obs_ptr[L];
    if (int rc = c->d_loo.alloc(c, pTot + 2 * nobs + (size_t)L)) return rc;
    std::vector<RowNormTask> rows;
    std::vector<LooTask> lt((size_t)L);
    for (int l = 0; l < L; ++l) {
        const LeafHost& lf = c->leaves[l];
        const LeafHost& ow = c->leaves[lf.owner];
        lt[l].P = c->d_loo.p + poff[lf.owner];
        lt[l].alpha = c->h_leaves[c->grad_src[l] >= 0 ? c->grad_src[l] : l].alpha;
        lt[l].off = (long long)c->obs_ptr[l];
        lt[l].ldp = ow.npad;
        if (lf.owner != l) continue;
        for (int t = 0; t * TB < lf.n; ++t)
            for (int c0 = t * TB, k = 0; c0 < lf.n; c0 += ROWNORM_COLS, ++k) {
                RowNormTask r{};
                r.X = c->arenaX + c->gxoff[l] + (size_t)t * TB;
                r.out = c->d_loo.p + poff[l] + (size_t)k * lf.npad + (size_t)t * TB;
                r.ld = lf.npad;
                r.col0 = c0;
                r.col1 = std::min(c0 + ROWNORM_COLS, lf.n);
                r.nrows = std::min(TB, lf.n - t * TB);
                rows.push_back(r);
            }
    }
    if (int rc = dev_upload(c, c->lrow, rows)) return rc;
    if (int rc = dev_upload(c, c->lleaf, lt)) return rc;
    c->loo_ready = true;
    return 0;
}
}

int dsmgp_loo(dsmgp_ctx* c, double* mu_out, double* var_out, double* lpd_out, double* seconds) {
    if (!c) return DSMGP_E_ARG;
    if (seconds) *seconds = 0.0;
    if (!c->fitted) return fail(c, DSMGP_E_STATE, "loo before fit");
    HIPCHK(c, hipSetDevice(c->device));
    const int L = c->L;
    OwnGradLists own_lists{c};
    if (int rc = xinv_lists(c, own_lists)) return rc;
    if (!c->loo_ready)
        if (int rc = build_loo_plan(c)) return rc;
    EventPair ev;
    HIPCHK(c, ev.init());
    HIPCHK(c, hipEventRecord(ev.a, c->stream));
    if (int rc = ensure_dinv(c)) return rc;
    if (int rc = ensure_alpha(c)) return rc;
    if (int rc = xinv_fill(c)) return rc;
    const size_t nobs = (size_t)c->obs_ptr[L];
    double* dmu = c->d_loo.p + (c->d_loo.count - 2 * nobs - (size_t)L);
    double* dvar = dmu + nobs;
    double* dlpd = dvar + nobs;
    if (c->lrow.count) rownorm_kernel<<<(unsigned)c->lrow.count, 256, 0, c->stream>>>(c->lrow.p);
    loo_moments_kernel<<<L, 256, 0, c->stream>>>(c->d_leaves.p, c->lleaf.p, c->d_obs_idx.p, c->dy.p, dmu, dvar, dlpd);
    HIPCHK(c, hipGetLastError());
    HIPCHK(c, hipEventRecord(ev.b, c->stream));
    HIPCHK(c, hipStreamSynchronize(c->stream));
    c->xinv_all = true;
    float ms = 0.f;
    HIPCHK(c, hipEventElapsedTime(&ms, ev.a, ev.b));
    if (seconds) *seconds = ms * 1e-3;
    if (mu_out) HIPCHK(c, hipMemcpy(mu_out, dmu, nobs * sizeof(double), hipMemcpyDeviceToHost));
    if (var_out) HIPCHK(c, hipMemcpy(var_out, dvar, nobs * sizeof(double), hipMemcpyDeviceToHost));
    if (lpd_out) HIPCHK(c, hipMemcpy(lpd_out, dlpd, (size_t)L * sizeof(double), hipMemcpyDeviceToHost));
    return 0;
}

int dsmgp_predict_gradients(dsmgp_ctx* c, double* dmu_out, double* dvar_out, int64_t ld, double* seconds) {
    if (!c) return DSMGP_E_ARG;
    if (seconds) *seconds = 0.0;
    if (!c->predicted || !c->vt_valid) return fail(c, DSMGP_E_STATE, "predict_gradients before predict_run on the current fit");
    const size_t nr = (size_t)c->route_total;
    if (nr == 0) return 0;
    if (ld < c->route_total) return fail(c, DSMGP_E_ARG, "predict_gradients: ld < route_total");
    HIPCHK(c, hipSetDevice(c->device));
    const int L = c->L, D = c->D;
    const bool var = dvar_out != nullptr;
    OwnGradLists own_lists{c};
    std::vector<size_t> boff((size_t)L, 0);
    if (var) {
        if (int rc = xinv_lists(c, own_lists)) return rc;
        size_t bTot = 0;
        for (int l = 0; l < L; ++l) {
            const LeafHost& lf = c->leaves[l];
            if (lf.nt == 0) continue;
            boff[l] = bTot;
            bTot += (size_t)lf.ntpad * lf.npad;
        }
        if (int rc = slab_grow(c, c->arenaB, c->cap_B, bTot)) return rc;
    }
    const size_t planes = (var ? 2 : 1) * (size_t)D * TB;
    std::vector<PredBetaTask> beta;
    std::vector<PredGradTask> tasks;
    std::vector<PredGradFinTask> fin;
    for (int l = 0; l < L; ++l) {
        const LeafHost& lf = c->leaves[l];
        if (lf.nt == 0) continue;
        const int nslab = (lf.n + PGRAD_SLAB - 1) / PGRAD_SLAB;
        for (int i = 0; i < lf.ntpad / TB; ++i) {
            PredGradFinTask f{};
            f.nslab = nslab;
            f.nrows = std::min(TB, lf.nt - i * TB);
            fin.push_back(f);
            for (int s = 0; s < nslab; ++s) tasks.push_back(PredGradTask{});
        }
    }
    if (int rc = c->d_pgpart.grow(c, tasks.size() * planes)) return rc;
    if (int rc = c->d_pgout.grow(c, (var ? 2 : 1) * nr * (size_t)D)) return rc;
    size_t ti = 0, fi = 0;
    for (int l = 0; l < L; ++l) {
        const LeafHost& lf = c->leaves[l];
        if (lf.nt == 0) continue;
        const LeafDev& d = c->h_leaves[l];
        const int nslab = (lf.n + PGRAD_SLAB - 1) / PGRAD_SLAB;
        double* Bl = var ? c->arenaB + boff[l] : nullptr;
        for (int i = 0; i < lf.ntpad / TB; ++i) {
            PredGradFinTask& f = fin[fi++];
            f.part = c->d_pgpart.p + ti * planes;
            f.xt = d.Xtg + (size_t)i * TB;
            f.dmu = c->d_pgout.p + (size_t)lf.route_off + (size_t)i * TB;
            f.dvar = var ? f.dmu + nr * (size_t)D : nullptr;
            f.info = d.info;
            f.pstride = (long long)planes;
            f.ldo = (long long)nr;
            f.ldt = lf.ntpad;
            f.kid = lf.kid;
            for (int s = 0; s < nslab; ++s) {
                PredGradTask& g = tasks[ti];
                g.xt = f.xt;
                g.xg = d.Xg;
                g.alpha = d.alpha;
                g.B = var ? Bl + (size_t)i * TB : nullptr;
                g.part = c->d_pgpart.p + ti * planes;
                g.ldt = lf.ntpad;
                g.ldg = lf.npad;
                g.nrows = f.nrows;
                g.c0 = s * PGRAD_SLAB;
                g.c1 = std::min(lf.n, g.c0 + PGRAD_SLAB);
                g.kid = lf.kid;
                ++ti;
            }
            if (!var) continue;
            const LeafHost& ow = c->leaves[lf.owner];
            for (int j = 0; j * TB < lf.n; ++j) {
                PredBetaTask b{};
                b.gemm.A = d.Vt + (size_t)i * TB;
// ... 304 lines not shown
        } else if (h.kind == DSMGP_KIND_ISO_LINEAR) {
            g[0] = -2.0 * (trMKy - cc * trM);
            g[1] = 0.0;
        } else if (h.kind == DSMGP_KIND_ARD_LINEAR) {
            for (int d = 0; d < nl; ++d)
                g[d] = -2.0 * (U[s * D + d] * A[s * D + d] - Q[s * D + d]) / std::exp(2.0 * h.loghyp[d]);
            g[nl] = 0.0;
        } else {
            if (KINDS[h.kind].iso_matern) {
                double sl = 0.0;
                for (int d = 0; d < D; ++d) sl += Sd[s * D + d];
                g[0] = sl;
            } else {
                for (int d = 0; d < nl; ++d) g[d] = Sd[s * D + d];
            }
            g[nl] = 2.0 * SK[s];
        }
        g[nl + 1] = 2.0 * noise * trM;
    }
    if (lpd_out) std::memcpy(lpd_out, lpd.data(), (size_t)L * sizeof(double));
    return 0;
}

int dsmgp_kernel_matrix(dsmgp_ctx* c, int32_t kernel_id, const double* x1, int64_t n1, const double* x2,
                        int64_t n2, double* K_out) {
    if (!c) return DSMGP_E_ARG;
    if (!x1 || !x2 || !K_out || n1 <= 0 || n2 <= 0 || c->D <= 0) return fail(c, DSMGP_E_ARG, "kernel_matrix: bad arguments");
    if (kernel_id < 0 || kernel_id >= (int)c->hyper.size() || c->hyper[kernel_id].kind < 0)
        return fail(c, DSMGP_E_STATE, "kernel_matrix: kernel id without hyper-parameters");
    if (ard_linear_short(c, kernel_id))
        return fail(c, DSMGP_E_ARG, std::string("kernel_matrix: ") + KINDS[c->hyper[kernel_id].kind].name +
                                        " needs one lengthscale per input dimension");
    HIPCHK(c, hipSetDevice(c->device));
    if (int rc = upload_hyper(c)) return rc;
    const int D = c->D;
    const int p1 = round_up((int)n1, TB), p2 = round_up((int)n2, TB);
    DevBuf<double> dx1, dx2, dK;
    if (int rc = dx1.alloc(c, (size_t)n1 * D)) return rc;
    if (int rc = dx2.alloc(c, (size_t)n2 * D)) return rc;
    if (int rc = dK.alloc(c, (size_t)p1 * p2)) return rc;
    HIPCHK(c, hipMemcpy(dx1.p, x1, (size_t)n1 * D * sizeof(double), hipMemcpyHostToDevice));
    HIPCHK(c, hipMemcpy(dx2.p, x2, (size_t)n2 * D * sizeof(double), hipMemcpyHostToDevice));
    std::vector<GramTask> g;
    for (int j = 0; j < p2 / TB; ++j)
        for (int i = 0; i < p1 / TB; ++i) {
            GramTask t{};
            t.xa = dx1.p + (size_t)i * TB;
            t.xb = dx2.p + (size_t)j * TB;
            t.out = dK.p + (size_t)i * TB + (size_t)j * TB * p1;
            t.lda = (int)n1;
            t.ldb = (int)n2;
            t.ldo = p1;
            t.na = (int)std::min<int64_t>(TB, n1 - (int64_t)i * TB);
            t.nb = (int)std::min<int64_t>(TB, n2 - (int64_t)j * TB);
            t.kid = kernel_id;
            g.push_back(t);
        }
    DevBuf<GramTask> dg;
    if (int rc = dev_upload(c, dg, g)) return rc;
    gram_tile_kernel<<<2 * (int)g.size(), 256, 0, c->stream>>>(dg.p, c->d_kp.p, D);
    HIPCHK(c, hipGetLastError());
    HIPCHK(c, hipStreamSynchronize(c->stream));
    HIPCHK(c, hipMemcpy2D(K_out, (size_t)n1 * sizeof(double), dK.p, (size_t)p1 * sizeof(double), (size_t)n1 * sizeof(double),
                          (size_t)n2, hipMemcpyDeviceToHost));
    return 0;
}

int dsmgp_download_factor(dsmgp_ctx* c, int32_t leaf, double* F, double* alpha) {
    if (!c) return DSMGP_E_ARG;
    if (!c->fitted) return fail(c, DSMGP_E_STATE, "download_factor before fit");
    if (leaf < 0 || leaf >= c->L) return fail(c, DSMGP_E_ARG, "leaf out of range");
    HIPCHK(c, hipSetDevice(c->device));
    const LeafHost& lf = c->leaves[leaf];
    const LeafDev& d = c->h_leaves[leaf];
    if (F) {
        HIPCHK(c, hipMemcpy2D(F, (size_t)lf.n * sizeof(double), d.F, (size_t)lf.npad * sizeof(double),
                              (size_t)lf.n * sizeof(double), (size_t)lf.n, hipMemcpyDeviceToHost));
        for (int col = 1; col < lf.n; ++col)
            for (int r = 0; r < col; ++r) F[r + (size_t)col * lf.n] = 0.0;
    }
    if (alpha) {
        if (int rc = ensure_alpha(c)) return rc;
        HIPCHK(c, hipMemcpy(alpha, d.alpha, lf.n * sizeof(double), hipMemcpyDeviceToHost));
    }
    return 0;
}

int dsmgp_timings(dsmgp_ctx* c, double* out) {
    if (!c || !out) return DSMGP_E_ARG;
    for (int i = 0; i < DSMGP_N_TIMINGS; ++i) out[i] = c->timings[i];
    return 0;
}

int dsmgp_work_gradients(dsmgp_ctx* c, double* alg_flops_inverse, double* alg_flops_contraction, int32_t* n_contraction_tiles) {
    if (!c) return DSMGP_E_ARG;
    double fi = 0.0, fc = 0.0;
    for (int l = 0; l < c->L; ++l) {
        const LeafHost& lf = c->leaves[l];
        const double n = (double)lf.n;
        if (lf.owner == l) fi += n * n * n / 3.0;
        if (lf.kid < (int)c->hyper.size() && c->hyper[lf.kid].kind >= 0 && KINDS[c->hyper[lf.kid].kind].contraction)
            fc += n * n * n / 3.0;
    }
    if (alg_flops_inverse) *alg_flops_inverse = fi;
    if (alg_flops_contraction) *alg_flops_contraction = fc;
    if (n_contraction_tiles) *n_contraction_tiles = (int32_t)c->gdot.count;
    return 0;
}

int dsmgp_work(dsmgp_ctx* c, double* alg_flops_update, int32_t* n_update_launches) {
    if (!c) return DSMGP_E_ARG;
    if (alg_flops_update) *alg_flops_update = c->last_fit_joint ? c->alg_flops_joint : c->alg_flops_update;
    if (n_update_launches) *n_update_launches = c->n_update_launches;
    return 0;
}

int dsmgp_lanes(dsmgp_ctx* c, int32_t* lanes) {
    if (!c || !lanes) return DSMGP_E_ARG;
    *lanes = c->plan_ready ? c->nlanes : 0;
    return 0;
}

int dsmgp_work_fused(dsmgp_ctx* c, double* alg_flops_fused, int32_t* n_fused_launches) {
    if (!c) return DSMGP_E_ARG;
    if (alg_flops_fused) *alg_flops_fused = c->last_fit_joint ? c->alg_flops_fused_joint : c->alg_flops_fused;
    if (n_fused_launches) *n_fused_launches = c->n_fused_launches;
    return 0;
}

int dsmgp_reserve(dsmgp_ctx* c, int64_t bytes) {
    if (!c || bytes < 0) return DSMGP_E_ARG;
    HIPCHK(c, hipSetDevice(c->device));
    HIPCHK(c, hipStreamSynchronize(c->stream));
    free_plan(c);
    free_test(c);
    if (c->pool_base) (void)hipFree(c->pool_base);
    c->pool_base = nullptr;
    c->pool_cap = c->pool_top = c->pool_mark_plan = 0;
    if (bytes == 0) return 0;
    void* p = nullptr;
    if (hipMalloc(&p, (size_t)bytes) != hipSuccess) {
        (void)hipGetLastError();
        return fail(c, DSMGP_E_NOMEM, "cannot reserve " + std::to_string(bytes >> 20) + " MiB of device memory");
    }
    c->pool_base = static_cast<char*>(p);
    c->pool_cap = (size_t)bytes;
    return 0;
}

int dsmgp_release(dsmgp_ctx* c) {
    if (!c) return DSMGP_E_ARG;
    HIPCHK(c, hipSetDevice(c->device));
    HIPCHK(c, hipStreamSynchronize(c->stream));
    HostLog hl("release");
    free_plan(c);
    free_test(c);
    return 0;
}

int64_t dsmgp_estimate_bytes(int32_t L, const int64_t* n, const int64_t* n_test, int32_t D, int32_t with_gradients) {
    int64_t tot = 0;
    for (int l = 0; l < L; ++l) {
        const int64_t np_ = (n[l] + TB - 1) / TB * TB;
        const int64_t nt_ = n_test ? (n_test[l] + TB - 1) / TB * TB : 0;
        tot += np_ * np_ * (with_gradients ? 2 : 1) + np_ * TB + np_ * (D + 4) + nt_ * np_ + nt_ * (D + 4);
    }
// ... 644 lines not shown
```

deepstructuredmixtures_amd/csrc/host_tree.cpp:

```cpp
#include "../../include/dsmgp_hip.h"
#include "route_walk.hpp"

#include <algorithm>
#include <atomic>
#include <cmath>
#include <cstdint>
#include <cstring>
#include <limits>
#include <memory>
#include <thread>
#include <vector>

#include <pthread.h>
#include <sched.h>
#include <unistd.h>

namespace {
int allowed_cpus(std::vector<int>* list = nullptr) {
    cpu_set_t set;
    CPU_ZERO(&set);
    int n = 0;
    if (sched_getaffinity(0, sizeof(set), &set) == 0)
        for (int c = 0; c < CPU_SETSIZE; ++c)
            if (CPU_ISSET(c, &set)) {
// ... 35 lines not shown
inline void offer(MainCand& m, double prod, int32_t leaf, int32_t count) {
    if (prod > m.prod || (prod == m.prod && m.prod > 0.0 && leaf < m.leaf)) m = MainCand{prod, leaf, count};
}
template <class CT>
void overlap_main_impl(int32_t L, const int64_t* obs_ptr, const int64_t* obs_idx, const std::vector<int64_t>& pptr,
                       const std::vector<int32_t>& pleaf, int nthr, int64_t* main_out, int64_t* c_main_out) {
    std::vector<std::vector<MainCand>> tabs((size_t)nthr);
    std::atomic<int32_t> next{0};
    const int32_t chunk = 16;
    auto work = [&](int t) {
        std::vector<MainCand>& tab = tabs[(size_t)t];
        tab.assign((size_t)L, MainCand{0.0, 0, 0});
        std::vector<CT> cnt((size_t)L, 0);
        std::vector<int32_t> touched;
        for (;;) {
            const int32_t j0 = next.fetch_add(chunk);
            if (j0 >= L) break;
            const int32_t j1 = std::min(L, j0 + chunk);
            for (int32_t j = j0; j < j1; ++j) {
                touched.clear();
                for (int64_t e = obs_ptr[j]; e < obs_ptr[j + 1]; ++e) {
                    const int64_t p = obs_idx[e];
                    for (int64_t q = pptr[p + 1] - 1; q >= pptr[p]; --q) {
                        const int32_t l = pleaf[q];
                        if (l <= j) break;
                        if (cnt[l]++ == 0) touched.push_back(l);
                    }
                }
                const double nj = (double)(obs_ptr[j + 1] - obs_ptr[j]);
                for (int32_t l : touched) {
                    const int32_t c = (int32_t)cnt[l];
                    cnt[l] = 0;
                    const double nl = (double)(obs_ptr[l + 1] - obs_ptr[l]);
                    const double d_jl = 1.0 - (nj - (double)c) / nj;
                    const double d_lj = 1.0 - (nl - (double)c) / nl;
                    const double prod = d_lj * d_jl;
                    offer(tab[(size_t)j], prod, l, c);
                    offer(tab[(size_t)l], prod, j, c);
                }
            }
        }
    };
    run_spread(nthr, work);
    for (int32_t j = 0; j < L; ++j) {
        MainCand m{0.0, 0, 0};
        for (int t = 0; t < nthr; ++t) {
            const MainCand& c = tabs[(size_t)t][(size_t)j];
            if (c.prod > 0.0) offer(m, c.prod, c.leaf, c.count);
        }
        main_out[j] = m.prod > 0.0 ? m.leaf : 0;
        c_main_out[j] = m.prod > 0.0 ? m.count : 0;
    }
}
}

extern "C" int dsmgp_overlap_main(int32_t L, const int64_t* obs_ptr, const int64_t* obs_idx, int64_t N, int64_t* main_out,
                       int64_t* c_main_out) {
    if (L < 0 || !obs_ptr || (!obs_idx && L > 0 && obs_ptr[L] > 0) || N <= 0 || !main_out || !c_main_out) return DSMGP_E_ARG;
    const int64_t total = L ? obs_ptr[L] : 0;
    int64_t nmax = 0;
    for (int32_t l = 0; l < L; ++l) {
        if (obs_ptr[l + 1] < obs_ptr[l]) return DSMGP_E_ARG;
        nmax = std::max(nmax, obs_ptr[l + 1] - obs_ptr[l]);
    }
    for (int64_t e = 0; e < total; ++e)
        if (obs_idx[e] < 0 || obs_idx[e] >= N) return DSMGP_E_ARG;
    std::vector<int64_t> pptr(N + 1, 0);
    for (int64_t e = 0; e < total; ++e) pptr[obs_idx[e] + 1]++;
    for (int64_t p = 0; p < N; ++p) pptr[p + 1] += pptr[p];
    std::vector<int32_t> pleaf(total);
    {
        std::vector<int64_t> fill(pptr.begin(), pptr.end() - 1);
        for (int32_t l = 0; l < L; ++l)
            for (int64_t e = obs_ptr[l]; e < obs_ptr[l + 1]; ++e) pleaf[fill[obs_idx[e]]++] = l;
    }
    const int64_t by_mem = std::max<int64_t>(1, (int64_t)(256u << 20) / std::max<int64_t>(1, (int64_t)L * (int64_t)sizeof(MainCand)));
    const int nthr = (int)std::max<int64_t>(1, std::min<int64_t>({16, (int64_t)allowed_cpus(), (int64_t)L / 512 + 1, by_mem}));
    if (nmax < 65536) overlap_main_impl<uint16_t>(L, obs_ptr, obs_idx, pptr, pleaf, nthr, main_out, c_main_out);
    else overlap_main_impl<int32_t>(L, obs_ptr, obs_idx, pptr, pleaf, nthr, main_out, c_main_out);
    return 0;
}

namespace {
#pragma clang fp contract(off)

static double np_pairwise(const double* a, int64_t n) {
    if (n < 8) {
        double r = -0.0;
        for (int64_t i = 0; i < n; ++i) r += a[i];
        return r;
    }
    if (n <= 128) {
        double r[8];
        for (int j = 0; j < 8; ++j) r[j] = a[j];
        int64_t i = 8;
        for (; i < n - (n % 8); i += 8)
            for (int j = 0; j < 8; ++j) r[j] += a[i + j];
        double res = ((r[0] + r[1]) + (r[2] + r[3])) + ((r[4] + r[5]) + (r[6] + r[7]));
        for (; i < n; ++i) res += a[i];
        return res;
    }
    int64_t n2 = n / 2;
    n2 -= n2 % 8;
    return np_pairwise(a, n2) + np_pairwise(a + n2, n - n2);
}

static double np_sum(const double* a, int64_t n) {
    constexpr int64_t NP_BUFSIZE = 8192;
    double out = 0.0;
    for (int64_t i = 0; i < n; i += NP_BUFSIZE) out += np_pairwise(a + i, std::min(NP_BUFSIZE, n - i));
    return out;
}

struct TreeBuild {
    const double* X;
    std::vector<double> Xr;
    int64_t N;
    int D, minData, K, V, maxDepth, nKernels;
    double bnoise;
    bool sumRoot;
    uint64_t seed, pos = 0;
    std::vector<int32_t> kind, split_dim, parent;
    std::vector<double> lb, ub;
    std::vector<int64_t> thr_ptr, obs_ptr;
    std::vector<double> thr, dir_u;
    std::vector<int32_t> obs;
    std::unique_ptr<double[]> vals, sel, sel2;
    std::unique_ptr<int32_t[]> key;
    std::unique_ptr<uint16_t[]> bucket;
    struct RowStack {
        std::vector<std::unique_ptr<int32_t[]>> block;
        std::vector<size_t> cap;
        size_t cur = 0, top = 0;
        int32_t* push(size_t n) {
            while (cur < block.size() && top + n > cap[cur]) {
                ++cur;
                top = 0;
            }
            if (cur == block.size()) {
                const size_t c = std::max<size_t>(n, (size_t)1 << 20);
                block.emplace_back(new int32_t[c]);
                cap.push_back(c);
                top = 0;
            }
            int32_t* p = block[cur].get() + top;
            top += n;
            return p;
        }
    } rows;

    double rand() {
        uint64_t z = seed + (pos + 1) * 0x9E3779B97F4A7C15ull;
        ++pos;
        z = (z ^ (z >> 30)) * 0xBF58476D1CE4E5B9ull;
        z = (z ^ (z >> 27)) * 0x94D049BB133111EBull;
        z = z ^ (z >> 31);
        return (double)(z >> 11) * (1.0 / 9007199254740992.0);
    }
    double beta22() {
        double a = rand(), b = rand(), c = rand();
        if (a > b) std::swap(a, b);
        if (b > c) std::swap(b, c);
        if (a > b) std::swap(a, b);
        return b;
    }
    int new_node(int k, int par, const std::vector<double>& l, const std::vector<double>& u) {
// ... 375 lines not shown
```

deepstructuredmixtures_amd/hipabi.py:

```python
import ctypes as C
import os
import sys
import numpy as np

_HERE = os.path.dirname(os.path.abspath(__file__))
LIB_PATH = os.path.join(_HERE, "libdsmgp_hip.so")

N_TIMINGS = 21
AGG_MIXTURE, AGG_POE, AGG_GPOE, AGG_RBCM = 0, 1, 2, 3
OPT_ARD_LENGTHSCALE_GRADIENT = 1
OPT_FUSED_GRAM = 2
OPT_FUSED_STEPS = 3
OPT_DIAG_IN_UPDATE = 4
OPT_FIT_GRAPH = 5
OPT_LANES = 6
SCORE_NAMES = ("mse", "sse", "mae", "sae", "nlpd")


def agg_width(family, n_groups=0):
    return 3 if family == AGG_MIXTURE else (2 * int(n_groups) if family == AGG_RBCM else 2)
TIMING_NAMES = ("gram", "chol_update", "chol_diag", "chol_trsm", "solve", "mll", "predict_gram",
                "predict_update", "predict_trsm", "predict_var", "gradients", "total_fit", "total_predict", "chol_reduce", "alpha",
                "grad_inverse", "grad_contraction", "grad_traces", "chol_fused", "chol_update_union", "chol_fused_union")

_dp = C.POINTER(C.c_double)
_ip = C.POINTER(C.c_int32)
_lp = C.POINTER(C.c_int64)
_ctx = C.c_void_p

SIGNATURES = {
    "dsmgp_create": (C.c_int, [C.c_int32, C.POINTER(_ctx)]),
    "dsmgp_destroy": (C.c_int, [_ctx]),
    "dsmgp_last_error": (C.c_char_p, [_ctx]),
    "dsmgp_device_name": (C.c_int, [_ctx, C.c_char_p, C.c_int32]),
    "dsmgp_set_train": (C.c_int, [_ctx, _dp, _dp, C.c_int64, C.c_int32]),
    "dsmgp_set_leaves": (C.c_int, [_ctx, C.c_int32, _lp, _lp, _ip, _dp]),
    "dsmgp_set_sharing": (C.c_int, [_ctx, _ip, _ip, _lp]),
    "dsmgp_set_hyper": (C.c_int, [_ctx, C.c_int32, C.c_int32, _dp, C.c_int32]),
    "dsmgp_fit": (C.c_int, [_ctx, _dp, _ip, _dp]),
    "dsmgp_set_test": (C.c_int, [_ctx, _dp, C.c_int64, C.c_int32, _lp, _lp]),
    "dsmgp_set_tree": (C.c_int, [_ctx, C.c_int64, C.POINTER(C.c_int8), _lp, _lp, _lp, _dp, C.c_int64, _lp]),
    "dsmgp_set_test_routed": (C.c_int, [_ctx, _dp, C.c_int64, C.c_int32]),
    "dsmgp_routes": (C.c_int, [_ctx, _lp, _lp]),
    "dsmgp_predict_run": (C.c_int, [_ctx, _dp]),
    "dsmgp_predict_fetch": (C.c_int, [_ctx, _dp, _dp]),
    "dsmgp_predict_leaves": (C.c_int, [_ctx, _dp, C.c_int64, C.c_int32, _lp, _lp, _dp, _dp]),
    "dsmgp_predict_cov": (C.c_int, [_ctx, C.c_int32, C.c_int32, _dp, C.c_int64, _dp]),
    "dsmgp_predict_gradients": (C.c_int, [_ctx, _dp, _dp, C.c_int64, _dp]),
    "dsmgp_gradients": (C.c_int, [_ctx, _dp, C.c_int32]),
    "dsmgp_loo": (C.c_int, [_ctx, _dp, _dp, _dp, _dp]),
    "dsmgp_loo_gradients": (C.c_int, [_ctx, _dp, C.c_int32, _dp, _dp]),
    "dsmgp_set_gradient_leaves": (C.c_int, [_ctx, _ip]),
    "dsmgp_set_option": (C.c_int, [_ctx, C.c_int32, C.c_int32]),
    "dsmgp_lanes": (C.c_int, [_ctx, _ip]),
    "dsmgp_aggregate": (C.c_int, [_ctx, C.c_int32, _dp, _ip, C.c_int32, C.c_int32, C.c_int32, _dp, _dp]),
    "dsmgp_aggregate_partial": (C.c_int, [_ctx, C.c_int32, _dp, _ip, C.c_int32, _dp]),
    "dsmgp_aggregate_finish": (C.c_int, [_ctx, _dp, C.c_int32, C.c_int32, _dp, _dp]),
    "dsmgp_scores": (C.c_int, [_ctx, _dp, _dp]),
    "dsmgp_kernel_matrix": (C.c_int, [_ctx, C.c_int32, _dp, C.c_int64, _dp, C.c_int64, _dp]),
    "dsmgp_download_factor": (C.c_int, [_ctx, C.c_int32, _dp, _dp]),
    "dsmgp_set_profile": (C.c_int, [_ctx, C.c_int32]),
    "dsmgp_set_joint": (C.c_int, [_ctx, C.c_int32]),
    "dsmgp_timings": (C.c_int, [_ctx, _dp]),
    "dsmgp_work": (C.c_int, [_ctx, _dp, _ip]),
    "dsmgp_work_fused": (C.c_int, [_ctx, _dp, _ip]),
    "dsmgp_work_gradients": (C.c_int, [_ctx, _dp, _dp, _ip]),
    "dsmgp_release": (C.c_int, [_ctx]),
    "dsmgp_reserve": (C.c_int, [_ctx, C.c_int64]),
    "dsmgp_overlap_main": (C.c_int, [C.c_int32, _lp, _lp, C.c_int64, _lp, _lp]),
    "dsmgp_comm_unique_id": (C.c_int, [C.c_char_p]),
    "dsmgp_comm_init": (C.c_int, [_ctx, C.c_int32, C.c_int32, C.c_char_p]),
    "dsmgp_allgather": (C.c_int, [_ctx, _dp, C.c_int64, _dp]),
    "dsmgp_fit_exchange": (C.c_int, [_ctx, C.c_int64, _dp]),
    "dsmgp_aggregate_exchange": (C.c_int, [_ctx, _dp]),
    "dsmgp_aggregate_exchange_empty": (C.c_int, [_ctx, C.c_int32, C.c_int64, _dp]),
    "dsmgp_comm_destroy": (C.c_int, [_ctx]),
    "dsmgp_tree_build": (C.c_int, [_dp, C.c_int64, C.c_int32, C.c_int32, C.c_int32, C.c_int32, C.c_int32, C.c_double, C.c_int32,
                                   C.c_int32, C.c_uint64, C.POINTER(C.c_void_p)]),
    "dsmgp_tree_sizes": (C.c_int, [C.c_void_p, _lp, _lp, _lp, _lp]),
    "dsmgp_tree_export": (C.c_int, [C.c_void_p, _ip, _ip, _ip, _dp, _dp, _lp, _dp, _lp, _lp, _dp]),
    "dsmgp_tree_means": (C.c_int, [C.c_void_p, _dp, C.c_int64, _dp]),
    "dsmgp_tree_free": (C.c_int, [C.c_void_p]),
    "dsmgp_tree_route": (C.c_int, [C.c_int64, C.POINTER(C.c_int8), _lp, _lp, _lp, _dp, C.c_int64, _lp, C.c_int64, _dp, C.c_int64,
                                   C.c_int64, C.c_int64, C.c_int64, _lp, _lp, C.c_int64, _lp]),
    "dsmgp_estimate_bytes": (C.c_int64, [C.c_int32, _lp, _lp, C.c_int32, C.c_int32]),
    "dsmgp_memory": (C.c_int, [_ctx, _lp, _lp]),
    "dsmgp_probe_f64_mfma": (C.c_int, [_ctx, _dp]),
    "dsmgp_probe_f64_mfma_detail": (C.c_int, [_ctx, C.c_int32, _dp]),
    "dsmgp_clock_sample_start": (C.c_int, [_ctx, C.c_double]),
    "dsmgp_clock_sample_read": (C.c_int, [_ctx, _dp, _dp]),
}

DIAG_SIGNATURES = {
    "dsmgp_probe_coissue": (C.c_int, [_ctx, _dp]),
    "dsmgp_bench_tile": (C.c_int, [_ctx, C.c_int32, C.c_int32, C.c_int32, C.c_int32, C.c_int32, _dp]),
    "dsmgp_probe_diag": (C.c_int, [_ctx, C.c_int32, C.c_int32, C.c_int32, _dp, _dp]),
    "dsmgp_bench_fused8": (C.c_int, [_ctx, C.c_int32, C.c_int32, C.c_int32, C.c_int32, _dp]),
    "dsmgp_probe_diag_fused": (C.c_int, [_ctx, C.c_int32, C.c_int32, C.c_int32, _dp]),
}
DIAG_LIB_PATH = os.path.join(_HERE, "libdsmgp_hip_diag.so")

_lib = None
_diag_lib = None


E_ARG, E_STATE, E_HIP, E_NOMEM, E_NODEVICE, E_DOMAIN = -1, -2, -3, -4, -5, -6


class DsmgpError(RuntimeError):
    def __init__(self, code, msg):
        super().__init__(f"dsmgp error {code}: {msg}")
        self.code = code


class DsmgpDomainError(DsmgpError, ValueError):
    """DSMGP_E_DOMAIN: a test row outside the region of a split node -- the ValueError the host routing raises for the same row."""


def load_diag_library():
    global _diag_lib
# ... 27 lines not shown

def _f64(a):
    a = np.ascontiguousarray(a, dtype=np.float64)
    return a, a.ctypes.data_as(_dp)


def _f64_fortran(a):
    a = np.asfortranarray(a, dtype=np.float64)
    return a, a.ctypes.data_as(_dp)


def _i64(a):
    a = np.ascontiguousarray(a, dtype=np.int64)
    return a, a.ctypes.data_as(_lp)


def _i32(a):
    a = np.ascontiguousarray(a, dtype=np.int32)
    return a, a.ctypes.data_as(_ip)


class Context:

    def __init__(self, device=0, diag=False):
        self.lib = load_diag_library() if diag else load_library()
        self.h = _ctx()
        rc = self.lib.dsmgp_create(int(device), C.byref(self.h))
        if rc != 0:
            msg = self.lib.dsmgp_last_error(None).decode()
            self.h = None
            raise DsmgpError(rc, msg)
        self.L = 0
        self.n_obs = 0
        self.D = 0
        self.route_total = 0
        self.n_t = 0

    def _chk(self, rc):
        if rc != 0:
            raise (DsmgpDomainError if rc == E_DOMAIN else DsmgpError)(rc, self.lib.dsmgp_last_error(self.h).decode())

    def close(self):
        if self.h is not None:
            self.lib.dsmgp_destroy(self.h)
            self.h = None

    def __del__(self):
        try:
            self.close()
        except Exception:
            pass

    def device_name(self):
        buf = C.create_string_buffer(256)
        self._chk(self.lib.dsmgp_device_name(self.h, buf, 256))
        return buf.value.decode()

    def set_train(self, X, y):
        X, px = _f64_fortran(X)
        y, py = _f64(y)
        assert X.ndim == 2 and y.shape == (X.shape[0],)
        self._chk(self.lib.dsmgp_set_train(self.h, px, py, X.shape[0], X.shape[1]))
        self.D = X.shape[1]

    def set_leaves(self, obs_ptr, obs_idx, kernel_id, mean):
        obs_ptr, p0 = _i64(obs_ptr)
        obs_idx, p1 = _i64(obs_idx)
        kernel_id, p2 = _i32(kernel_id)
        mean, p3 = _f64(mean)
        L = len(obs_ptr) - 1
        self._chk(self.lib.dsmgp_set_leaves(self.h, L, p0, p1, p2, p3))
        self.L = L
        self.n_obs = int(obs_ptr[-1])

    def set_sharing(self, op, src, plen):
        if op is None:
            self._chk(self.lib.dsmgp_set_sharing(self.h, None, None, None))
            return
        op, p0 = _i32(op)
        src, p1 = _i32(src)
        plen, p2 = _i64(plen)
        self._chk(self.lib.dsmgp_set_sharing(self.h, p0, p1, p2))

    def set_hyper(self, kernel_id, kind, loghyp):
        v, p = _f64(loghyp)
        self._chk(self.lib.dsmgp_set_hyper(self.h, int(kernel_id), int(kind), p, len(v)))

    def fit(self):
        mll = np.empty(self.L)
        info = np.empty(self.L, dtype=np.int32)
        sec = C.c_double(0.0)
        self._chk(self.lib.dsmgp_fit(self.h, mll.ctypes.data_as(_dp), info.ctypes.data_as(_ip), C.byref(sec)))
        return mll, info, sec.value

    def _test_matrix(self, Xt):
        Xt, px = _f64_fortran(Xt)
        if Xt.ndim != 2 or Xt.shape[1] != self.D:
            raise ValueError(f"test matrix of shape {Xt.shape}: the model was trained on D = {self.D} columns")
        return Xt, px

    def set_test(self, Xt, route_ptr, route_idx):
        Xt, px = self._test_matrix(Xt)
        route_ptr, p0 = _i64(route_ptr)
        route_idx, p1 = _i64(route_idx)
        self._chk(self.lib.dsmgp_set_test(self.h, px, Xt.shape[0], Xt.shape[1], p0, p1))
        self.route_total = int(route_ptr[-1])
        self.n_t = int(Xt.shape[0])

    def set_tree(self, kind, first_child, n_child, split_dim, thr, leaf_local):
        kind = np.ascontiguousarray(kind, dtype=np.int8)
        first_child, p1 = _i64(first_child)
        n_child, p2 = _i64(n_child)
        split_dim, p3 = _i64(split_dim)
        thr = np.ascontiguousarray(thr, dtype=np.float64)
        leaf_local, p5 = _i64(leaf_local)
        self._chk(self.lib.dsmgp_set_tree(self.h, int(kind.size), kind.ctypes.data_as(C.POINTER(C.c_int8)), p1, p2, p3,
                                          thr.ctypes.data_as(_dp), int(thr.shape[1]), p5))

    def set_test_routed(self, Xt):
        Xt, px = self._test_matrix(Xt)
        self._chk(self.lib.dsmgp_set_test_routed(self.h, px, Xt.shape[0], Xt.shape[1]))
        self.n_t = int(Xt.shape[0])
        ptr = np.zeros(self.L + 1, dtype=np.int64)
        self._chk(self.lib.dsmgp_routes(self.h, ptr.ctypes.data_as(_lp), None))
        self.route_total = int(ptr[-1])
        return ptr

    def routes(self):
        ptr = np.zeros(self.L + 1, dtype=np.int64)
        self._chk(self.lib.dsmgp_routes(self.h, ptr.ctypes.data_as(_lp), None))
        idx = np.zeros(max(1, int(ptr[-1])), dtype=np.int64)
        self._chk(self.lib.dsmgp_routes(self.h, ptr.ctypes.data_as(_lp), idx.ctypes.data_as(_lp)))
        return ptr, idx[:int(ptr[-1])]

    def predict_run(self):
        sec = C.c_double(0.0)
        self._chk(self.lib.dsmgp_predict_run(self.h, C.byref(sec)))
        return sec.value

    def predict_fetch(self):
        mu = np.empty(self.route_total)
        var = np.empty(self.route_total)
        self._chk(self.lib.dsmgp_predict_fetch(self.h, mu.ctypes.data_as(_dp), var.ctypes.data_as(_dp)))
        return mu, var

    def predict_leaves(self, Xt, route_ptr, route_idx):
        self.set_test(Xt, route_ptr, route_idx)
        self.predict_run()
        return self.predict_fetch()

    def predict_cov(self, leaf, nt, with_noise=True):
        nt = int(nt)
        S = np.empty((nt, nt), dtype=np.float64, order="F")
        sec = C.c_double(0.0)
        self._chk(self.lib.dsmgp_predict_cov(self.h, int(leaf), 1 if with_noise else 0, S.ctypes.data_as(_dp), nt, C.byref(sec)))
        self.cov_seconds = sec.value
        return S

    def predict_gradients(self, want_var=True):
        n = int(self.route_total)
        dmu = np.empty((n, self.D), dtype=np.float64, order="F")
        dvar = np.empty((n, self.D), dtype=np.float64, order="F") if want_var else None
        sec = C.c_double(0.0)
        self._chk(self.lib.dsmgp_predict_gradients(self.h, dmu.ctypes.data_as(_dp),
                                                   dvar.ctypes.data_as(_dp) if want_var else None, max(1, n), C.byref(sec)))
        self.grad_seconds = sec.value
# ... 177 lines not shown
    def probe_f64_mfma_detail(self, blocks_per_cu=4):
        out = np.zeros(4)
        self._chk(self.lib.dsmgp_probe_f64_mfma_detail(self.h, int(blocks_per_cu), out.ctypes.data_as(_dp)))
        return dict(zip(("tflops", "cycles_per_mfma", "clock_ghz", "waves_per_simd"), out.tolist()))

    def clock_sample_start(self, milliseconds):
        self._chk(self.lib.dsmgp_clock_sample_start(self.h, float(milliseconds)))

    def clock_sample_read(self):
        g, ms = C.c_double(0.0), C.c_double(0.0)
        self._chk(self.lib.dsmgp_clock_sample_read(self.h, C.byref(g), C.byref(ms)))
        return g.value, ms.value

    def probe_coissue(self):
        out = np.zeros(9)
        self._chk(self.lib.dsmgp_probe_coissue(self.h, out.ctypes.data_as(_dp)))
        return {m: dict(mfma_tflops=out[3 * i], valu_tflops=out[3 * i + 1], ms=out[3 * i + 2])
                for i, m in enumerate(("mfma_only", "valu_only", "both"))}

    def probe_diag(self, ntiles, ld=8192, reps=20):
        us = C.c_double(0.0)
        ph = np.zeros(23)
        self._chk(self.lib.dsmgp_probe_diag(self.h, int(ntiles), int(ld), int(reps), C.byref(us), ph.ctypes.data_as(_dp)))
        return us.value, ph

    def probe_diag_fused(self, ntiles, K=0, reps=10):
        us = C.c_double(0.0)
        self._chk(self.lib.dsmgp_probe_diag_fused(self.h, int(ntiles), int(K), int(reps), C.byref(us)))
        return us.value

    def bench_tile(self, ntiles, K, mode=0, group=16, reps=3):
        s = C.c_double(0.0)
        self._chk(self.lib.dsmgp_bench_tile(self.h, int(ntiles), int(K), int(mode), int(group), int(reps), C.byref(s)))
        return 2.0 * 128 * 128 * K * ntiles / s.value / 1e12

    def bench_fused8(self, ntasks, K, group=16, reps=3):
        s = C.c_double(0.0)
        self._chk(self.lib.dsmgp_bench_fused8(self.h, int(ntasks), int(K), int(group), int(reps), C.byref(s)))
        return s.value

    def probe_f64_mfma(self):
        t = C.c_double(0.0)
        self._chk(self.lib.dsmgp_probe_f64_mfma(self.h, C.byref(t)))
        return t.value


class MultiContext:

    def __init__(self, device=0, n=2):
        from concurrent.futures import ThreadPoolExecutor
        self.subs = [Context(device) for _ in range(n)]
        self.pool = ThreadPoolExecutor(max_workers=n)
        self.L = 0
        self.route_total = 0
        self._leaves = None
        self._sharing = (None, None, None)
        self._dirty = True
        self._test = None
        self._test_dirty = False
        self.part = None
        self.act = self.subs

    def close(self):
        for s in self.subs:
            s.close()
        self.pool.shutdown(wait=False)

    def device_name(self):
        return self.subs[0].device_name()

    def _each(self, fn):
        return list(self.pool.map(fn, self.act))

    def set_train(self, X, y):
        for s in self.subs:
            s.set_train(X, y)
        self._dirty = True

    def set_leaves(self, obs_ptr, obs_idx, kernel_id, mean):
        self._leaves = (np.asarray(obs_ptr, dtype=np.int64), np.asarray(obs_idx, dtype=np.int64),
                        np.asarray(kernel_id, dtype=np.int32), np.asarray(mean, dtype=np.float64))
        self.L = len(obs_ptr) - 1
        self._sharing = (None, None, None)
        self._dirty = True
        self._test = None

    def set_sharing(self, op, src, plen):
        self._sharing = (None, None, None) if op is None else (np.asarray(op), np.asarray(src), np.asarray(plen))
        self._dirty = True

    def set_hyper(self, kernel_id, kind, loghyp):
        for s in self.subs:
            s.set_hyper(kernel_id, kind, loghyp)

    def set_joint(self, on):
        for s in self.subs:
            s.set_joint(on)

    def set_option(self, option, value):
        for s in self.subs:
            s.set_option(option, value)
        self._test_dirty = self._test is not None

    def set_profile(self, on):
        for s in self.subs:
            s.set_profile(on)

    def _partition(self):
        ptr = self._leaves[0]
        n = np.diff(ptr).astype(np.float64)
        op, src, _ = self._sharing
        group = np.arange(self.L)
        if op is not None:
            for j in range(self.L):
                if op[j] != 0 and src[j] >= 0:
                    group[j] = src[j]
        cost = np.zeros(self.L)
        for j in range(self.L):
            cost[group[j]] += n[j] ** 3 if (op is None or op[j] == 0) else n[j] ** 2
        load = np.zeros(len(self.subs))
        owner_of = {}
        for g in sorted(set(group.tolist()), key=lambda g: -cost[g]):
            r = int(np.argmin(load))
            owner_of[g] = r
            load[r] += cost[g]
        owner = np.array([owner_of[g] for g in group])
        return [np.flatnonzero(owner == r) for r in range(len(self.subs))]

    def _upload(self):
        if not self._dirty:
            return
        ptr, idx, kid, mean = self._leaves
        op, src, plen = self._sharing
        parts = self._partition()
        self.act = [s for s, loc in zip(self.subs, parts) if len(loc)]
        self.part = [loc for loc in parts if len(loc)]
        for s, loc in zip(self.act, self.part):
            lptr = np.concatenate([[0], np.cumsum(ptr[loc + 1] - ptr[loc])])
            lidx = np.concatenate([idx[ptr[g]:ptr[g + 1]] for g in loc]) if len(loc) else np.zeros(0, np.int64)
            s.set_leaves(lptr, lidx, kid[loc], mean[loc])
            if op is None:
                s.set_sharing(None, None, None)
            else:
                g2l = {int(g): i for i, g in enumerate(loc)}
                s.set_sharing(op[loc], np.array([g2l.get(int(src[g]), -1) for g in loc], dtype=np.int32), plen[loc])
        self._dirty = False
        self._test_dirty = self._test is not None

    def _upload_test(self):
        if not self._test_dirty:
            return
        Xt, rptr, ridx = self._test
        for s, loc in zip(self.act, self.part):
            lptr = np.concatenate([[0], np.cumsum(rptr[loc + 1] - rptr[loc])])
            lidx = np.concatenate([ridx[rptr[g]:rptr[g + 1]] for g in loc]) if len(loc) else np.zeros(0, np.int64)
            s.set_test(Xt, lptr, lidx)
        self._test_dirty = False

    def fit(self):
        self._upload()
        self._upload_test()
        res = self._each(lambda s: s.fit())
        mll = np.empty(self.L)
        info = np.empty(self.L, dtype=np.int32)
        for (m, i, _), loc in zip(res, self.part):
            mll[loc] = m
            info[loc] = i
        return mll, info, max(r[2] for r in res)

    def set_test(self, Xt, route_ptr, route_idx):
        self._test = (np.asfortranarray(Xt, dtype=np.float64), np.asarray(route_ptr, dtype=np.int64),
                      np.asarray(route_idx, dtype=np.int64))
        self.route_total = int(route_ptr[-1])
        self._test_dirty = True
        if not self._dirty:
            self._upload_test()

    def predict_run(self):
        self._upload()
        self._upload_test()
        return max(self._each(lambda s: s.predict_run()))

    def predict_fetch(self):
        _, rptr, _ = self._test
        mu = np.empty(self.route_total)
        var = np.empty(self.route_total)
        for s, loc in zip(self.act, self.part):
            m, v = s.predict_fetch()
            pos = 0
            for g in loc:
                c = int(rptr[g + 1] - rptr[g])
                mu[rptr[g]:rptr[g + 1]] = m[pos:pos + c]
                var[rptr[g]:rptr[g + 1]] = v[pos:pos + c]
                pos += c
        return mu, var

    def predict_leaves(self, Xt, route_ptr, route_idx):
        self.set_test(Xt, route_ptr, route_idx)
        self.predict_run()
        return self.predict_fetch()

    def predict_cov(self, leaf, nt, with_noise=True):
        raise DsmgpError(E_STATE, "predict_cov: the full covariance of a leaf is served by a single Context only "
                                  "(MultiContext spreads the leaf table over several devices)")

    def predict_gradients(self, want_var=True):
        _, rptr, _ = self._test
        res = self._each(lambda s: s.predict_gradients(want_var))
        D = self.act[0].D
        dmu = np.empty((self.route_total, D), dtype=np.float64, order="F")
        dvar = np.empty((self.route_total, D), dtype=np.float64, order="F") if want_var else None
        for (m, v), loc in zip(res, self.part):
            pos = 0
            for g in loc:
                c = int(rptr[g + 1] - rptr[g])
                dmu[rptr[g]:rptr[g + 1]] = m[pos:pos + c]
                if want_var:
                    dvar[rptr[g]:rptr[g + 1]] = v[pos:pos + c]
                pos += c
        self.grad_seconds = max(s.grad_seconds for s in self.act)
        return dmu, dvar

    def aggregate_partial(self, family, leaf_coef=None, leaf_group=None, n_groups=0):
        coef = None if leaf_coef is None else np.asarray(leaf_coef, dtype=np.float64)
        grp = None if leaf_group is None else np.asarray(leaf_group, dtype=np.int32)
        tot = None
        for s, loc in zip(self.act, self.part):
            p = s.aggregate_partial(family, None if coef is None else coef[loc], None if grp is None else grp[loc], n_groups)
# ... 103 lines not shown
                              ptr.ctypes.data_as(_lp), idx.ctypes.data_as(_lp), int(idx.size), C.byref(nr))
    if rc != 0:
        if rc == -1 and split_dim.size and x.shape[1] <= int(split_dim.max()):
            raise IndexError(f"test rows have {x.shape[1]} columns, the tree splits on dimension {int(split_dim.max())}")
        raise ValueError("test point outside the region of a split node (reference loops forever here)" if rc == E_DOMAIN
                         else f"dsmgp_tree_route failed ({rc}): malformed tree arrays")
    return ptr, idx[:nr.value].copy() if nr.value < idx.size else idx


def tree_build(X, min_data, n_splits, n_sum_children, depth, bnoise, sum_root, n_kernels, seed, y=None):
    lib = load_library()
    X, px = _f64_fortran(X)
    N, D = X.shape
    h = C.c_void_p()
    rc = lib.dsmgp_tree_build(px, N, D, int(min_data), int(n_splits), int(n_sum_children), int(depth), float(bnoise),
                              1 if sum_root else 0, int(n_kernels), C.c_uint64(int(seed)), C.byref(h))
    if rc != 0:
        raise DsmgpError(rc, "dsmgp_tree_build: bad arguments (non-finite inputs?)")
    try:
        n, nthr, nobs, ndir = (C.c_int64(0) for _ in range(4))
        lib.dsmgp_tree_sizes(h, C.byref(n), C.byref(nthr), C.byref(nobs), C.byref(ndir))
        n, nthr, nobs, ndir = n.value, nthr.value, nobs.value, ndir.value
        out = dict(kind=np.empty(n, np.int32), parent=np.empty(n, np.int32), split_dim=np.empty(n, np.int32),
                   lb=np.empty((n, D)), ub=np.empty((n, D)), thr_ptr=np.empty(n + 1, np.int64), thr=np.empty(max(nthr, 1)),
                   obs_ptr=np.empty(n + 1, np.int64), obs=np.empty(max(nobs, 1), np.int64), dir_u=np.empty(max(ndir, 1)))
        rc = lib.dsmgp_tree_export(h, out["kind"].ctypes.data_as(_ip), out["parent"].ctypes.data_as(_ip),
                                   out["split_dim"].ctypes.data_as(_ip), out["lb"].ctypes.data_as(_dp), out["ub"].ctypes.data_as(_dp),
                                   out["thr_ptr"].ctypes.data_as(_lp), out["thr"].ctypes.data_as(_dp),
                                   out["obs_ptr"].ctypes.data_as(_lp), out["obs"].ctypes.data_as(_lp), out["dir_u"].ctypes.data_as(_dp))
        if rc != 0:
            raise DsmgpError(rc, "dsmgp_tree_export failed")
        out["thr"], out["obs"], out["dir_u"] = out["thr"][:nthr], out["obs"][:nobs], out["dir_u"][:ndir]
        if y is not None:
            y = np.ascontiguousarray(y, dtype=np.float64)
            if y.shape != (N,):
                raise ValueError("tree_build: y must have one value per row of X")
            out["mean"] = np.empty(max(int(np.count_nonzero(out["kind"] == 0)), 1))
            rc = lib.dsmgp_tree_means(h, y.ctypes.data_as(_dp), N, out["mean"].ctypes.data_as(_dp))
            if rc != 0:
                raise DsmgpError(rc, "dsmgp_tree_means failed")
        return out
    finally:
        lib.dsmgp_tree_free(h)


class StreamingContext:

    def __init__(self, device=0, budget_bytes=None, headroom=0.85):
        self.ctx = Context(device)
        self.budget = budget_bytes
        self.headroom = headroom
        self.L = 0
        self.D = 0
        self.route_total = 0
        self._leaves = None
        self._sharing = (None, None, None)
        self._hyper = {}
        self._test = None
        self.want_gradients = 0
        self.keep_alpha = ()
        self.groups = None
        self._res = None
        self.passes = 0
        self._pool_bytes = 0
        self._auto_budget = None
        self.verbose = bool(os.environ.get("DSMGP_STREAM_VERBOSE"))

    def close(self):
        self.ctx.close()

    def device_name(self):
        return self.ctx.device_name()

    def set_train(self, X, y):
        self.ctx.set_train(X, y)
        self.D = np.asarray(X).shape[1]
        self._res = None

    def set_leaves(self, obs_ptr, obs_idx, kernel_id, mean):
        self._leaves = (np.asarray(obs_ptr, dtype=np.int64), np.asarray(obs_idx, dtype=np.int64),
                        np.asarray(kernel_id, dtype=np.int32), np.asarray(mean, dtype=np.float64))
        self.L = len(obs_ptr) - 1
        self._sharing = (None, None, None)
        self._test = None
        self.groups = None
        self._res = None

    def set_sharing(self, op, src, plen):
        self._sharing = (None, None, None) if op is None else (np.asarray(op), np.asarray(src), np.asarray(plen))
        self.groups = None
        self._res = None

    def set_hyper(self, kernel_id, kind, loghyp):
        self.ctx.set_hyper(kernel_id, kind, loghyp)
        self._res = None

    def set_joint(self, on):
        pass

    def set_option(self, option, value):
        self.ctx.set_option(option, value)
        self._res = None

    def set_profile(self, on):
        self.ctx.set_profile(on)

    def set_test(self, Xt, route_ptr, route_idx):
        self._test = (np.asfortranarray(Xt, dtype=np.float64), np.asarray(route_ptr, dtype=np.int64),
                      np.asarray(route_idx, dtype=np.int64))
        self.route_total = int(route_ptr[-1])
        self.groups = None
        self._res = None

    def _make_groups(self):
        ptr = self._leaves[0]
        n = np.diff(ptr)
        nt = np.diff(self._test[1]) if self._test is not None else np.zeros(self.L, dtype=np.int64)
        op, src, _ = self._sharing
        unit = np.arange(self.L)
        if op is not None:
            for j in range(self.L):
                if op[j] != 0 and src[j] >= 0:
                    unit[j] = src[j]
        budget = self.budget
        if budget is None:
            if self._pool_bytes:
                budget = self._auto_budget
            else:
                budget = self._auto_budget = int(self.ctx.memory()[1] * self.headroom)
        units = {}
        for j in range(self.L):
            units.setdefault(int(unit[j]), []).append(j)
        sized = []
        for u, members in units.items():
            m = np.array(members)
            own = m if op is None else m[op[m] != 1]
            b = estimate_bytes(n[own], nt[own], self.D, bool(self.want_gradients))
            if op is not None and np.any(op[m] == 1):
                cp = m[op[m] == 1]
                b += int(np.sum((nt[cp] + 128) * (n[cp] + 128) * 8))
            sized.append((b, members))
        sized.sort(key=lambda t: -t[0])
        if sized and sized[0][0] > budget:
            raise DsmgpError(-4, f"one leaf group needs {sized[0][0] >> 20} MiB, budget is {budget >> 20} MiB")
        groups, loads = [], []
        for b, members in sized:
            for gi in range(len(groups)):
                if loads[gi] + b <= budget:
                    groups[gi].extend(members)
                    loads[gi] += b
                    break
            else:
                groups.append(list(members))
                loads.append(b)
        self.groups = [np.array(sorted(g)) for g in groups]
        want = 0 if len(self.groups) < 2 else int(max(loads)) + (3 << 30)
        if want != self._pool_bytes:
            self.ctx.reserve(want)
            self._pool_bytes = want

    def _pass(self):
        if self.groups is None:
            self._make_groups()
        ptr, idx, kid, mean = self._leaves
        op, src, plen = self._sharing
        mll = np.empty(self.L)
        info = np.zeros(self.L, dtype=np.int32)
        mu = np.empty(self.route_total)
        var = np.empty(self.route_total)
        grads = np.zeros((self.L, self.want_gradients)) if self.want_gradients else None
        alphas = {}
        seconds, tpred = 0.0, 0.0
        tsum = {}
        flops, launches = 0.0, 0
        fflops, flaunches = 0.0, 0
        import time as _time
        host = {"set_leaves": 0.0, "set_sharing": 0.0, "set_test": 0.0, "fit": 0.0, "release": 0.0}

        def timed(key, fn, *a):
            t0 = _time.perf_counter()
            r = fn(*a)
            host[key] += _time.perf_counter() - t0
            return r

        t_pass = _time.perf_counter()
        for gi, loc in enumerate(self.groups):
            if self.verbose:
                print(f"# streaming pass {self.passes + 1}: group {gi + 1}/{len(self.groups)} ({len(loc)} leaves) at "
                      f"{_time.perf_counter() - t_pass:.1f} s", file=sys.stderr, flush=True)
            c = self.ctx
            lptr = np.concatenate([[0], np.cumsum(ptr[loc + 1] - ptr[loc])])
            timed("set_leaves", c.set_leaves, lptr, np.concatenate([idx[ptr[g]:ptr[g + 1]] for g in loc]), kid[loc], mean[loc])
            if op is None:
                timed("set_sharing", c.set_sharing, None, None, None)
            else:
                g2l = {int(g): i for i, g in enumerate(loc)}
                timed("set_sharing", c.set_sharing, op[loc],
                      np.array([g2l.get(int(src[g]), -1) for g in loc], dtype=np.int32), plen[loc])
            if self._test is not None:
                Xt, rptr, ridx = self._test
                tptr = np.concatenate([[0], np.cumsum(rptr[loc + 1] - rptr[loc])])
                timed("set_test", c.set_test, Xt, tptr, np.concatenate([ridx[rptr[g]:rptr[g + 1]] for g in loc]))
            m, i, s = timed("fit", c.fit)
            mll[loc], info[loc] = m, i
            seconds += s
            if self._test is not None:
                tpred += c.predict_run()
                gm, gv = c.predict_fetch()
                pos = 0
                for g in loc:
                    k = int(rptr[g + 1] - rptr[g])
                    mu[rptr[g]:rptr[g + 1]] = gm[pos:pos + k]
                    var[rptr[g]:rptr[g + 1]] = gv[pos:pos + k]
                    pos += k
            if self.want_gradients:
                grads[loc] = c.gradients(self.want_gradients)
            for g in self.keep_alpha:
                li = np.flatnonzero(loc == g)
                if li.size:
                    alphas[int(g)] = c.download_factor(int(li[0]), int(ptr[g + 1] - ptr[g]), factor=False)[1]
            for k_, v_ in c.timings().items():
                tsum[k_] = tsum.get(k_, 0.0) + v_
            f_, n_ = c.work()
            flops += f_
            launches += n_
            ff_, fn_ = c.work_fused()
            fflops += ff_
            flaunches += fn_
            timed("release", c.release)
        self.passes += 1
        self.host_seconds = host
        self._res = dict(mll=mll, info=info, mu=mu, var=var, grads=grads, seconds=seconds, tpred=tpred, timings=tsum,
                         work=(flops, launches), work_fused=(fflops, flaunches), has_test=self._test is not None, alpha=alphas)

    def fit(self):
        self._pass()
        r = self._res
        return r["mll"], r["info"], r["seconds"]

    def predict_run(self):
        if self._res is None or not self._res["has_test"]:
            self._pass()
        return self._res["tpred"]

    def predict_fetch(self):
        return self._res["mu"], self._res["var"]

    def predict_cov(self, leaf, nt, with_noise=True):
        raise DsmgpError(E_STATE, "predict_cov: a streaming pass discards K_tn L^-T with its leaf group; "
                                  "use a resident Context for the full covariance of a leaf")

    def predict_gradients(self, want_var=True):
        raise DsmgpError(E_STATE, "predict_gradients: a streaming pass discards alpha, K_tn L^-T and L^-T with their leaf group; "
                                  "use a resident Context for the input gradients of the prediction")

    def predict_leaves(self, Xt, route_ptr, route_idx):
        self.set_test(Xt, route_ptr, route_idx)
        self.predict_run()
        return self.predict_fetch()

    def set_gradient_leaves(self, active=None):
        return None

    def gradients(self, stride):
        if self._res is None or self._res["grads"] is None or self._res["grads"].shape[1] < stride:
            self.want_gradients = int(stride)
            self.groups = None
            self._pass()
        return self._res["grads"][:, :stride].copy()

    def loo(self):
        raise DsmgpError(E_STATE, "loo: a streaming pass discards the factors and L^-T with their leaf group; "
                                  "use a resident Context for leave-one-out moments")

    def loo_gradients(self, stride):
        raise DsmgpError(E_STATE, "loo_gradients: a streaming pass discards the factors and L^-T with their leaf group; "
                                  "use a resident Context for the gradients of the leave-one-out density")

    def timings(self):
        return dict(self._res["timings"]) if self._res else {k: 0.0 for k in TIMING_NAMES}

# ... 12 lines not shown
```

deepstructuredmixtures_amd/model.py:

```python
import numpy as np

try:
    import xxhash as _xxhash
except ImportError:
    _xxhash = None

from . import hipabi
from .kernels import (IsoSE, ConstMean, KIND_ISO_SE, KIND_ARD_SE, KIND_ISO_LINEAR, KIND_ARD_LINEAR, KIND_ARD_SE_PRODUCT,
                      KIND_ISO_MATERN32, KIND_ISO_MATERN52, KIND_ARD_MATERN32, KIND_ARD_MATERN52)
from .tree import (DSMGPConfig, GPSumNode, build_tree, get_leaves, get_overlap, obs_table, share_schedule, share_decisions,
                   share_census, route, route_all, route_index, get_child, ordered_nodes, SHARE_COPY, SHARE_FULL, SHARE_PREFIX)
from . import dist as _dist
from . import datagen as _datagen

EPS = 1e-8


def _logsumexp(a, axis=None):
    a = np.asarray(a, dtype=np.float64)
    if axis is None:
        m = np.max(a)
        m = m if np.isfinite(m) else 0.0
        return float(np.log(np.sum(np.exp(a - m))) + m)
    m = np.max(a, axis=axis, keepdims=True)
    m = np.where(np.isfinite(m), m, 0.0)
    return np.squeeze(np.log(np.sum(np.exp(a - m), axis=axis, keepdims=True)) + m, axis=axis)


class TreeIndex:

    def __init__(self, root):
        nodes, depth, parent_edge = [root], [0], [-1]
        levels = []
        frontier = [0]
        edge_child, edge_parent = [], []
        d = 0
        while frontier:
            par, seg, cnt, nxt = [], [], [], []
            e0 = len(edge_child)
            for ni in frontier:
                nd = nodes[ni]
                if nd.kind == "gp":
                    continue
                par.append(ni)
                seg.append(len(edge_child) - e0)
                cnt.append(len(nd.children))
                for c in nd.children:
                    nodes.append(c)
                    depth.append(d + 1)
                    parent_edge.append(len(edge_child))
                    edge_child.append(len(nodes) - 1)
                    edge_parent.append(ni)
                    nxt.append(len(nodes) - 1)
            if par:
                levels.append(dict(parent=np.array(par), seg=np.array(seg), cnt=np.array(cnt), e0=e0,
                                   e1=len(edge_child)))
            frontier = nxt
            d += 1
        self.nodes = nodes
        self.n = len(nodes)
        self.edge_child = np.array(edge_child, dtype=np.int64)
        self.edge_parent = np.array(edge_parent, dtype=np.int64)
        self.parent_edge = np.array(parent_edge, dtype=np.int64)
        is_sum = np.array([nd.kind == "sum" for nd in nodes])
        of_gps = np.array([nd.kind == "sum" and nd.of_gps for nd in nodes])
        nch = np.array([0 if nd.kind == "gp" else len(nd.children) for nd in nodes], dtype=np.float64)
        self.edge_is_sum = is_sum[self.edge_parent] if self.edge_parent.size else np.zeros(0, bool)
        self.edge_of_gps = of_gps[self.edge_parent] if self.edge_parent.size else np.zeros(0, bool)
        self.edge_prior = np.where(self.edge_is_sum, -np.log(np.maximum(nch[self.edge_parent], 1.0)), 0.0) \
            if self.edge_parent.size else np.zeros(0)
        self.leaf_node = np.array([i for i, nd in enumerate(nodes) if nd.kind == "gp"], dtype=np.int64)
        self.leaf_id = np.array([nodes[i].leaf for i in self.leaf_node], dtype=np.int64)
        for lv in levels:
            lv["parent_is_sum"] = is_sum[lv["parent"]]
        self.levels = levels
        self.lw = np.zeros(self.edge_child.size)
        self.bind()

    def bind(self):
        for lv in self.levels:
            for ni, a, k in zip(lv["parent"], lv["seg"] + lv["e0"], lv["cnt"]):
                nd = self.nodes[ni]
# ... 68 lines not shown
        self.share_branch = None
        self.fit_census = None

    @property
    def tindex(self):
        if self._tindex is None:
            self._tindex = TreeIndex(self.root)
        elif not self._tindex.bound():
            self._tindex.bind()
        return self._tindex

    @property
    def ctx(self):
        if self._ctx is None:
            if self._stream_budget is not None:
                b = None if self._stream_budget == "auto" else int(self._stream_budget)
                self._ctx = hipabi.StreamingContext(self._device, b)
            elif self._n_sub > 1:
                self._ctx = hipabi.MultiContext(self._device, self._n_sub)
            else:
                self._ctx = hipabi.Context(self._device)
                if self.shard.world > 1:
                    self.shard.device_comm(self._ctx)
        return self._ctx

    def kernel_table(self):
        if getattr(self, "_ktab", None) is None:
            tab = {}
            for lf in self.leaves:
                tab.setdefault(lf.kernelid, lf)
            self._ktab = [tab[k] for k in sorted(tab)]
        return self._ktab

    def _push_hyper(self):
        for lf in self.kernel_table():
            hyp = np.concatenate([lf.kernel.loghyp(), [lf.logNoise]])
            self.ctx.set_hyper(lf.kernelid, lf.kernel.kind, hyp)

    def set_option(self, option, value):
        self.ctx.set_option(option, value)
        if self._route_cache is not None:
            self._route_cache["uploaded"] = False

    def _set_decisions(self, dec):
        if dec is None:
            dec = (np.zeros(self.L, dtype=np.int32), np.full(self.L, -1, dtype=np.int32), np.zeros(self.L, dtype=np.int64),
                   np.zeros(self.L, dtype=np.int8))
        self.share_op, self.share_branch = dec[0], dec[3]
        self.fit_census = share_census(dec[3])
        return dec

    def _upload(self, tau):
        loc = self.shard.local
        key = ("sched", None if tau is None else float(tau))
        if self._uploaded and self._schedule == key:
            return
        if len(loc) == 0:
            self._uploaded = True
            self._schedule = key
            self._route_cache = None
            if self.D is not None and tau is not None:
                self._set_decisions(share_decisions(self.leaves, self.D, tau))
            else:
                self._set_decisions(None)
            return
        if not self._uploaded:
            self.ctx.set_train(self.x, self.y)
        lv = [self.leaves[i] for i in loc]
        ptr, idx = obs_table(lv)
        self.ctx.set_leaves(ptr, idx, [lf.kernelid for lf in lv], [lf.mean.m for lf in lv])
        if self.D is not None and tau is not None:
            op, src, plen, _ = self._set_decisions(share_decisions(self.leaves, self.D, tau))
            g2l = {g: i for i, g in enumerate(loc)}
            lop = np.zeros(len(lv), dtype=np.int32)
            lsrc = np.full(len(lv), -1, dtype=np.int32)
            lpl = np.zeros(len(lv), dtype=np.int64)
            for i, g in enumerate(loc):
                if op[g] != SHARE_FULL and int(src[g]) in g2l:
                    lop[i], lsrc[i], lpl[i] = op[g], g2l[int(src[g])], plen[g]
            self.ctx.set_sharing(lop, lsrc, lpl)
        else:
            self._set_decisions(None)
            self.ctx.set_sharing(None, None, None)
        self._uploaded = True
        self._schedule = key
        self._route_cache = None
        self._register_tree(loc)

    def _register_tree(self, loc):
        self._device_routing = False
        if self.family != "dsmgp" or self.root.kind == "gp" or not hasattr(self.ctx, "set_tree"):
            return
        ri = route_index(self.root)
        g2l = np.full(self.L, -1, dtype=np.int64)
        g2l[np.asarray(loc, dtype=np.int64)] = np.arange(len(loc))
        leaf_local = np.where(ri.leaf >= 0, g2l[np.maximum(ri.leaf, 0)], -1)
        try:
            self.ctx.set_tree(ri.kind, ri.first, ri.nchild, ri.sdim, ri.thr, leaf_local)
            self._device_routing = True
        except hipabi.DsmgpError:
            pass


class DSMGP(Model):
    family = "dsmgp"


class PoE(Model):
    family = "poe"


class gPoE(Model):
    family = "gpoe"


class rBCM(Model):
    family = "rbcm"



def build(x, y, K, V, eps, M, D, kernel, meanFun, logNoise, useSum, *, seed=7, device=0, ctx=None,
          cls=DSMGP, tau=0.05, fit_now=True, shard_world=None, n_sub=1, stream_budget=None):
    x = np.asarray(x, dtype=np.float64)
    if x.ndim == 1:
        x = x.reshape(-1, 1)
    config = DSMGPConfig(meanFun, kernel, logNoise, M, V, K, D, eps, useSum)
    root = build_tree(x, np.asarray(y, dtype=np.float64), config, seed=seed)
    L = len(get_leaves(root))
    overlap = get_overlap(root, L)
    model = cls(root, x, y, overlap, ctx=ctx, device=device, n_sub=n_sub, stream_budget=stream_budget)
    if shard_world is not None:
        rank, world = shard_world
        op, src, _ = share_schedule(model.leaves, overlap, tau)
        model.shard = _dist.Shard.lpt([lf.nobs for lf in model.leaves], op, src, rank, world)
    if fit_now:
        fit(model, tau=tau)
    return model


def buildDSMGP(x, y, K, V, *, eps=0.5, M=30, D=2, kernel=None, meanFun=None, logNoise=1.0, sum=True, **kw):
    kernel = IsoSE(1.0, 1.0) if kernel is None else kernel
    return build(x, y, K, V, eps, M, D, kernel, meanFun, logNoise, sum, cls=DSMGP, **kw)


def buildPoE(x, y, V, *, eps=0.0, M=30, D=2, kernel=None, meanFun, logNoise=1.0, generalized=False, **kw):
    kernel = IsoSE(1.0, 1.0) if kernel is None else kernel
    return build(x, y, 1, V, eps, M, D, kernel, meanFun, logNoise, False, cls=gPoE if generalized else PoE, **kw)


def buildBCM(x, y, V, *, eps=0.0, M=30, D=2, kernel=None, meanFun=None, logNoise=1.0, robust=False, **kw):
    kernel = IsoSE(1.0, 1.0) if kernel is None else kernel
    return build(x, y, 1, V, eps, M, D, kernel, meanFun, logNoise, False, cls=rBCM, **kw)


class GaussianProcess:

    def __init__(self, x, y, *, mean=None, kernel=None, logNoise=np.log(7.0), run_cholesky=False, device=0, ctx=None):
        from .tree import GPNode
        x = np.asarray(x, dtype=np.float64)
        if x.ndim == 1:
            x = x.reshape(-1, 1)
        y = np.asarray(y, dtype=np.float64)
        mean = ConstMean(float(np.mean(y))) if mean is None else mean
        kernel = IsoSE(0.0, 0.0) if kernel is None else kernel
        N, D = x.shape
        leaf = GPNode(np.arange(N), np.full(D, -np.inf), np.full(D, np.inf), kernel, 0, mean, logNoise)
# ... 1020 lines not shown
```

include/dsmgp_hip.h:

```cpp
#ifndef DSMGP_HIP_H
#define DSMGP_HIP_H

#include <stdint.h>

#ifdef __cplusplus
extern "C" {
#endif

typedef struct dsmgp_ctx dsmgp_ctx;

#define DSMGP_KIND_ISO_SE     0
#define DSMGP_KIND_ARD_SE     1
#define DSMGP_KIND_ISO_LINEAR 2
#define DSMGP_KIND_ARD_LINEAR 3
#define DSMGP_KIND_ARD_SE_PRODUCT 4
#define DSMGP_KIND_ISO_MATERN32 5
#define DSMGP_KIND_ISO_MATERN52 6
#define DSMGP_KIND_ARD_MATERN32 7
#define DSMGP_KIND_ARD_MATERN52 8

#define DSMGP_SHARE_FULL   0
#define DSMGP_SHARE_COPY   1
#define DSMGP_SHARE_PREFIX 2

#define DSMGP_OK            0
#define DSMGP_E_ARG        -1
#define DSMGP_E_STATE      -2
#define DSMGP_E_HIP        -3
#define DSMGP_E_NOMEM      -4
#define DSMGP_E_NODEVICE   -5
#define DSMGP_E_DOMAIN     -6

#define DSMGP_N_TIMINGS 21

#define DSMGP_MAX_KERNEL_IDS (1 << 22)

int dsmgp_create(int32_t device_id, dsmgp_ctx** out);
int dsmgp_destroy(dsmgp_ctx* ctx);
const char* dsmgp_last_error(dsmgp_ctx* ctx);
int dsmgp_device_name(dsmgp_ctx* ctx, char* buf, int32_t len);

int dsmgp_set_train(dsmgp_ctx* ctx, const double* X , const double* y ,
                    int64_t N, int32_t D);

int dsmgp_set_leaves(dsmgp_ctx* ctx, int32_t L, const int64_t* obs_ptr ,
                     const int64_t* obs_idx, const int32_t* kernel_id, const double* mean );

int dsmgp_set_sharing(dsmgp_ctx* ctx, const int32_t* op , const int32_t* src ,
                      const int64_t* prefix_len );

int dsmgp_set_hyper(dsmgp_ctx* ctx, int32_t kernel_id, int32_t kind, const double* loghyp, int32_t n);

int dsmgp_fit(dsmgp_ctx* ctx, double* mll_out , int32_t* info_out , double* seconds);

int dsmgp_set_joint(dsmgp_ctx* ctx, int32_t on);
int dsmgp_set_test(dsmgp_ctx* ctx, const double* Xt , int64_t n_t, int32_t D,
                   const int64_t* route_ptr , const int64_t* route_idx);
int dsmgp_set_tree(dsmgp_ctx* ctx, int64_t n_nodes, const int8_t* kind, const int64_t* first_child, const int64_t* n_child,
                   const int64_t* split_dim, const double* thr, int64_t thr_ld, const int64_t* leaf_id);
int dsmgp_set_test_routed(dsmgp_ctx* ctx, const double* Xt , int64_t n_t, int32_t D);
int dsmgp_routes(dsmgp_ctx* ctx, int64_t* route_ptr , int64_t* route_idx );
int dsmgp_predict_run(dsmgp_ctx* ctx, double* seconds);
int dsmgp_predict_fetch(dsmgp_ctx* ctx, double* mu_out, double* var_out);
int dsmgp_predict_leaves(dsmgp_ctx* ctx, const double* Xt, int64_t n_t, int32_t D, const int64_t* route_ptr,
                         const int64_t* route_idx, double* mu_out, double* var_out);
int dsmgp_predict_cov(dsmgp_ctx* ctx, int32_t leaf, int32_t with_noise, double* Sigma_out, int64_t ld, double* seconds);
int dsmgp_predict_gradients(dsmgp_ctx* ctx, double* dmu_out, double* dvar_out ,
                            int64_t ld, double* seconds);

#define DSMGP_AGG_MIXTURE 0
#define DSMGP_AGG_POE     1
#define DSMGP_AGG_GPOE    2
#define DSMGP_AGG_RBCM    3
int dsmgp_aggregate(dsmgp_ctx* ctx, int32_t family, const double* leaf_coef , const int32_t* leaf_group ,
                    int32_t n_groups, int32_t plain, int32_t prior_kernel_id, double* mu_out, double* var_out);
int dsmgp_aggregate_partial(dsmgp_ctx* ctx, int32_t family, const double* leaf_coef, const int32_t* leaf_group,
                            int32_t n_groups, double* partial_out );
int dsmgp_aggregate_finish(dsmgp_ctx* ctx, const double* partial_in , int32_t plain,
                           int32_t prior_kernel_id, double* mu_out, double* var_out);
int dsmgp_scores(dsmgp_ctx* ctx, const double* y_test , double* out );

int dsmgp_gradients(dsmgp_ctx* ctx, double* grad_out, int32_t stride);
int dsmgp_set_gradient_leaves(dsmgp_ctx* ctx, const int32_t* active );
int dsmgp_loo(dsmgp_ctx* ctx, double* mu_out, double* var_out ,
              double* lpd_out , double* seconds );
int dsmgp_loo_gradients(dsmgp_ctx* ctx, double* grad_out , int32_t stride,
                        double* lpd_out , double* seconds );
#define DSMGP_OPT_ARD_LENGTHSCALE_GRADIENT 1
#define DSMGP_OPT_FUSED_GRAM 2
#define DSMGP_OPT_FUSED_STEPS 3
#define DSMGP_OPT_DIAG_IN_UPDATE 4
#define DSMGP_OPT_FIT_GRAPH 5
#define DSMGP_OPT_LANES 6
int dsmgp_set_option(dsmgp_ctx* ctx, int32_t option, int32_t value);
int dsmgp_lanes(dsmgp_ctx* ctx, int32_t* lanes);

int dsmgp_kernel_matrix(dsmgp_ctx* ctx, int32_t kernel_id, const double* x1, int64_t n1,
                        const double* x2, int64_t n2, double* K_out );
int dsmgp_download_factor(dsmgp_ctx* ctx, int32_t leaf, double* F , double* alpha );
int dsmgp_set_profile(dsmgp_ctx* ctx, int32_t level);
int dsmgp_timings(dsmgp_ctx* ctx, double* out );
int dsmgp_work(dsmgp_ctx* ctx, double* alg_flops_update, int32_t* n_update_launches);
int dsmgp_work_fused(dsmgp_ctx* ctx, double* alg_flops_fused, int32_t* n_fused_launches);
int dsmgp_work_gradients(dsmgp_ctx* ctx, double* alg_flops_inverse, double* alg_flops_contraction, int32_t* n_contraction_tiles);
int dsmgp_reserve(dsmgp_ctx* ctx, int64_t bytes);

int dsmgp_release(dsmgp_ctx* ctx);
int64_t dsmgp_estimate_bytes(int32_t L, const int64_t* n, const int64_t* n_test , int32_t D,
                             int32_t with_gradients);
int dsmgp_memory(dsmgp_ctx* ctx, int64_t* needed, int64_t* free_bytes);

int dsmgp_probe_f64_mfma(dsmgp_ctx* ctx, double* tflops);
int dsmgp_probe_f64_mfma_detail(dsmgp_ctx* ctx, int32_t blocks_per_cu, double* out);

int dsmgp_clock_sample_start(dsmgp_ctx* ctx, double milliseconds);
int dsmgp_clock_sample_read(dsmgp_ctx* ctx, double* ghz, double* milliseconds);

int dsmgp_overlap_main(int32_t L, const int64_t* obs_ptr, const int64_t* obs_idx, int64_t N, int64_t* main_out,
                       int64_t* c_main_out);

int dsmgp_tree_route(int64_t n_nodes, const int8_t* kind, const int64_t* first_child, const int64_t* n_child,
                     const int64_t* split_dim, const double* thr, int64_t thr_ld, const int64_t* leaf_id, int64_t n_leaves,
                     const double* x, int64_t n_t, int64_t D, int64_t row_stride, int64_t col_stride, int64_t* route_ptr,
                     int64_t* route_idx, int64_t capacity, int64_t* n_routes_out);

int dsmgp_comm_unique_id(char* id_out );
int dsmgp_comm_init(dsmgp_ctx* ctx, int32_t rank, int32_t world, const char* id );
int dsmgp_allgather(dsmgp_ctx* ctx, const double* send, int64_t count, double* recv );
int dsmgp_fit_exchange(dsmgp_ctx* ctx, int64_t count, double* out );
int dsmgp_aggregate_exchange(dsmgp_ctx* ctx, double* total_out );
int dsmgp_aggregate_exchange_empty(dsmgp_ctx* ctx, int32_t W, int64_t n_t, double* total_out );
int dsmgp_comm_destroy(dsmgp_ctx* ctx);

typedef struct dsmgp_tree dsmgp_tree;
int dsmgp_tree_build(const double* X , int64_t N, int32_t D, int32_t min_data, int32_t n_splits,
                     int32_t n_sum_children, int32_t depth, double bnoise, int32_t sum_root, int32_t n_kernels, uint64_t seed,
                     dsmgp_tree** out);
int dsmgp_tree_sizes(const dsmgp_tree* t, int64_t* n_nodes, int64_t* n_thr, int64_t* n_obs, int64_t* n_dir);
int dsmgp_tree_export(const dsmgp_tree* t, int32_t* kind, int32_t* parent, int32_t* split_dim, double* lb, double* ub,
                      int64_t* thr_ptr, double* thr, int64_t* obs_ptr, int64_t* obs, double* dir_u);
int dsmgp_tree_means(const dsmgp_tree* t, const double* y, int64_t N, double* mean_out);
int dsmgp_tree_free(dsmgp_tree* t);

#ifdef __cplusplus
}
#endif
#endif
```

Baseline: 0.3851.

## Share Cholesky prefix factorization between overlapping leaves via row reordering

Adds a host-side planner that pairs eligible leaves with the same kernel that share many observations. It reorders each leaf's rows so the shared points form a common prefix, then marks one leaf as a prefix-sharer of the other, so the shared leading block of the Cholesky factor is computed only once. A separate forward-solve task list is added for the shared prefix blocks, and outputs are permuted back to caller order. The feature is enabled by default from model.py through an environment variable, with row limits. The cost is host-side planning, extra reordering and permutation, and added complexity in the fused-step and sharing logic.

```diff
diff --git a/deepstructuredmixtures_amd/csrc/dsmgp_hip.cpp b/deepstructuredmixtures_amd/csrc/dsmgp_hip.cpp
--- a/deepstructuredmixtures_amd/csrc/dsmgp_hip.cpp
+++ b/deepstructuredmixtures_amd/csrc/dsmgp_hip.cpp
@@ -38,6 +38,7 @@
     int64_t prefix = 0;
     int owner = -1;
     int kb = 0;
+    bool ovl = false;
     size_t f_off = 0, dinv_off = 0, vec_off = 0, xg_off = 0;
     int nt = 0, ntpad = 0;
     size_t vt_off = 0, xt_off = 0, pv_off = 0;
@@ -397,6 +398,13 @@
     std::vector<LeafHost> leaves;
     std::vector<int64_t> obs_ptr, obs_idx;
     DevBuf<int64_t> d_obs_ptr, d_obs_idx;
+    std::vector<int64_t> obs_int;
+    std::vector<int32_t> obs_cpos;
+    bool ovl_on = true;
+    int64_t ovl_max = 0;
+    int64_t ovl_min = 0;
+    int ovl_pairs = 0;
+    double ovl_saved = 0.0;
     bool plan_ready = false;
 
     std::vector<HyperHost> hyper;
@@ -441,8 +449,9 @@
     int tail_split = DSMGP_TAIL_SPLIT_DEFAULT, tail_rounds = DSMGP_TAIL_ROUNDS_DEFAULT;
     int tail_split_lanes = DSMGP_TAIL_SPLIT_LANES, tail_rounds_lanes = DSMGP_TAIL_ROUNDS_LANES;
     int ragged_rounds = 2, ragged_div = 4;
-    std::vector<int> fwd_off, bwd_off;
+    std::vector<int> fwd_off, bwd_off, fwd_pre_off;
     DevBuf<SolveTask> fwd, bwd;
+    DevBuf<SolveTask> fwd_pre;
     int solve_steps = 0;
     bool fitted = false;
     bool use_graph = false;
@@ -820,6 +829,7 @@
         for (auto& ph : lane) ph.drop(false);
     for (auto& sl : c->slabF) arena_put(c, sl);
     c->fwd.release();
+    c->fwd_pre.release();
     c->bwd.release();
     c->dinvc_prefix.release();
     c->dinvc_fwd.release();
@@ -1094,6 +1104,7 @@
                 if (lf.nb <= k || !in_phase(lf)) continue;
                 const LeafDev& d = c->h_leaves[l];
                 const int ld = lf.npad;
+                const bool zfit = ph != 1 || lf.ovl;
                 if (lf.owner == l) {
                     const int i_first = (k < lf.kb) ? lf.kb : k;
                     const bool own_diag = (k >= lf.kb);
@@ -1109,7 +1120,7 @@
                                 b.gx = d.Xg + (size_t)i * TB + r;
                                 b.lda = b.ldc = b.glda = ld;
                                 b.nvalid = std::min(16, rows - r);
-                                if (ph != 1) b.wi = d.w + (size_t)i * TB + r;
+                                if (zfit) b.wi = d.w + (size_t)i * TB + r;
                                 blocks8.push_back(b);
                             }
                             continue;
@@ -1167,7 +1178,7 @@
                             s.k1 = TB;
                             s.update = 0;
                             s.mrows = tile_mrows(lf.n - i * TB);
-                            if (ph != 1) {
+                            if (zfit) {
                                 s.zk = d.z + (size_t)k * TB;
                                 s.wi = d.w + (size_t)i * TB;
                             }
@@ -1178,7 +1189,7 @@
                         DiagTask g{};
                         g.T = d.F + (size_t)k * TB + (size_t)k * TB * ld;
                         g.Dinv = d.Dinv + (size_t)k * TB * TB;
-                        if (ph != 1) {
+                        if (zfit) {
                             g.wk = d.w + (size_t)k * TB;
                             g.zk = d.z + (size_t)k * TB;
                         }
@@ -1498,7 +1509,8 @@
             const LeafHost& lf = c->leaves[l];
             unit[l] = lf.op == DSMGP_SHARE_FULL ? l : lf.src;
             const double n = (double)lf.n;
-            cost[unit[l]] += lf.op == DSMGP_SHARE_COPY ? n * n : n * n * n;
+            const double p = lf.ovl ? (double)lf.prefix : 0.0;
+            cost[unit[l]] += lf.op == DSMGP_SHARE_COPY ? n * n : n * n * n - p * p * p;
         }
         int nunits = 0;
         for (int l = 0; l < L; ++l) nunits += unit[l] == l ? 1 : 0;
@@ -1585,7 +1597,7 @@
             if (lf.op == DSMGP_SHARE_PREFIX)
                 for (int k = 0; k < lf.kb; ++k)
                     if (fused_in(0, k)) pre.push_back(block_task(l, k));
-            if (lf.op == DSMGP_SHARE_FULL) continue;
+            if (lf.op == DSMGP_SHARE_FULL || lf.ovl) continue;
             const int o = lf.owner;
             if (done[o]) continue;
             done[o] = 1;
@@ -1611,17 +1623,21 @@
         int nsteps = 0;
         for (auto& lf : c->leaves) nsteps = std::max(nsteps, lf.nb);
         c->solve_steps = nsteps;
-        std::vector<SolveTask> fwd, bwd;
+        std::vector<SolveTask> fwd, bwd, pre;
         c->fwd_off.assign(nsteps + 1, 0);
         c->bwd_off.assign(nsteps + 1, 0);
+        c->fwd_pre_off.assign(nsteps + 1, 0);
         for (int k = 0; k < nsteps; ++k) {
             c->fwd_off[k] = (int)fwd.size();
+            c->fwd_pre_off[k] = (int)pre.size();
             for (int l = 0; l < L; ++l) {
                 const LeafHost& lf = c->leaves[l];
                 if (lf.nb <= k) continue;
                 if (lf.owner == l && lf.op == DSMGP_SHARE_FULL) continue;
+                if (lf.ovl && k >= lf.kb) continue;
                 const LeafDev& d = c->h_leaves[l];
-                for (int i = k; i < lf.nb; ++i) {
+                std::vector<SolveTask>& dst = lf.ovl ? pre : fwd;
+                for (int i = k; i < (lf.ovl ? lf.kb : lf.nb); ++i) {
                     SolveTask s{};
                     s.Dk = d.Dinv + (size_t)k * TB * TB;
                     s.vk = d.w + (size_t)k * TB;
@@ -1633,11 +1649,13 @@
                         s.T = d.F + (size_t)i * TB + (size_t)k * TB * lf.npad;
                         s.vi = d.w + (size_t)i * TB;
                     }
-                    fwd.push_back(s);
+                    dst.push_back(s);
                 }
             }
         }
         c->fwd_off[nsteps] = (int)fwd.size();
+        c->fwd_pre_off[nsteps] = (int)pre.size();
+        if (int rc = dev_upload(c, c->fwd_pre, pre)) return rc;
         for (int s_ = 0; s_ < nsteps; ++s_) {
             c->bwd_off[s_] = (int)bwd.size();
             for (int l = 0; l < L; ++l) {
@@ -1918,6 +1936,94 @@
     return 0;
 }
 
+extern "C" int dsmgp_overlap_plan(int32_t L, const int64_t* obs_ptr, const int64_t* obs_idx, const int32_t* kernel_id,
+                                  const int32_t* eligible, int64_t N, int64_t min_shared_rows, int32_t* src_out, int64_t* shared_out,
+                                  int64_t* order_out, int32_t* n_pairs, double* flops_saved);
+int apply_overlap(dsmgp_ctx* c) {
+    const int L = c->L;
+    const bool want = c->ovl_on && c->ovl_min > 0;
+    bool had = !c->obs_int.empty();
+    for (int l = 0; l < L; ++l) had = had || c->leaves[l].ovl;
+    if (!had && !want) return 0;
+    HIPCHK(c, hipSetDevice(c->device));
+    free_plan(c);
+    free_test(c);
+    for (int l = 0; l < L; ++l) {
+        LeafHost& lf = c->leaves[l];
+        if (!lf.ovl) continue;
+        lf.ovl = false;
+        lf.op = DSMGP_SHARE_FULL;
+        lf.src = -1;
+        lf.prefix = 0;
+    }
+    c->ovl_pairs = 0;
+    c->ovl_saved = 0.0;
+    std::vector<int64_t> order;
+    bool reordered = false;
+    if (want) {
+        std::vector<int32_t> elig((size_t)L, 1), kid((size_t)L), src((size_t)L);
+        std::vector<int64_t> shared((size_t)L);
+        for (int l = 0; l < L; ++l) {
+            const LeafHost& lf = c->leaves[l];
+            kid[(size_t)l] = lf.kid;
+            if (lf.op != DSMGP_SHARE_FULL || (c->ovl_max > 0 && lf.n > c->ovl_max)) elig[(size_t)l] = 0;
+            if (lf.op == DSMGP_SHARE_PREFIX) elig[(size_t)lf.src] = 0;
+        }
+        for (int l = 0; l < L; ++l) {
+            const LeafHost& lf = c->leaves[l];
+            if (lf.op == DSMGP_SHARE_COPY && elig[(size_t)lf.src] != 0) elig[(size_t)lf.src] = 2;
+        }
+        order.resize(c->obs_idx.size());
+        int32_t np = 0;
+        double saved = 0.0;
+        if (dsmgp_overlap_plan(L, c->obs_ptr.data(), c->obs_idx.data(), kid.data(), elig.data(), c->N, c->ovl_min, src.data(),
+                               shared.data(), order.data(), &np, &saved) != 0)
+            return fail(c, DSMGP_E_ARG, "plan_overlap_sharing: bad leaf table");
+        for (int l = 0; l < L; ++l) {
+            LeafHost& lf = c->leaves[l];
+            if (src[(size_t)l] >= 0) {
+                lf.ovl = true;
+                lf.op = DSMGP_SHARE_PREFIX;
+                lf.src = src[(size_t)l];
+                lf.prefix = shared[(size_t)l];
+            }
+        }
+        for (int l = 0; l < L; ++l) {
+            const LeafHost& lf = c->leaves[l];
+            if (lf.op == DSMGP_SHARE_COPY)
+                std::memcpy(order.data() + lf.obs_off, order.data() + c->leaves[lf.src].obs_off, sizeof(int64_t) * (size_t)lf.n);
+        }
+        c->ovl_pairs = np;
+        c->ovl_saved = saved;
+        reordered = order != c->obs_idx;
+    }
+    if (!reordered) {
+        if (!c->obs_int.empty())
+            HIPCHK(c, hipMemcpy(c->d_obs_idx.p, c->obs_idx.data(), c->obs_idx.size() * sizeof(int64_t), hipMemcpyHostToDevice));
+        c->obs_int.clear();
+        c->obs_cpos.clear();
+        return 0;
+    }
+    c->obs_int.swap(order);
+    c->obs_cpos.resize(c->obs_int.size());
+    for (int l = 0; l < L; ++l) {
+        const LeafHost& lf = c->leaves[l];
+        const int64_t* a = c->obs_idx.data() + lf.obs_off;
+        for (int i = 0; i < lf.n; ++i)
+            c->obs_cpos[(size_t)lf.obs_off + i] = (int32_t)(std::lower_bound(a, a + lf.n, c->obs_int[(size_t)lf.obs_off + i]) - a);
+    }
+    HIPCHK(c, hipMemcpy(c->d_obs_idx.p, c->obs_int.data(), c->obs_int.size() * sizeof(int64_t), hipMemcpyHostToDevice));
+    return 0;
+}
+
+void to_caller_order(const dsmgp_ctx* c, int l, double* v) {
+    if (c->obs_cpos.empty()) return;
+    const LeafHost& lf = c->leaves[l];
+    const int32_t* pos = c->obs_cpos.data() + lf.obs_off;
+    std::vector<double> t(v, v + lf.n);
+    for (int i = 0; i < lf.n; ++i) v[pos[i]] = t[(size_t)i];
+}
+
 }
 
 extern "C" {
@@ -2060,6 +2166,18 @@
         }
         c->diag_in_update = value != 0;
         return 0;
+    }
+    if (option == DSMGP_OPT_OVERLAP_SHARE) {
+        const bool on = value != 0;
+        if (on == c->ovl_on) return 0;
+        c->ovl_on = on;
+        return c->L > 0 ? apply_overlap(c) : 0;
+    }
+    if (option == DSMGP_OPT_OVERLAP_MAX_ROWS) {
+        if (value < 0) return fail(c, DSMGP_E_ARG, "set_option: the row limit must be 0 (none) or positive");
+        if (value == c->ovl_max) return 0;
+        c->ovl_max = value;
+        return c->L > 0 ? apply_overlap(c) : 0;
     }
     return fail(c, DSMGP_E_ARG, "set_option: unknown option");
 }
@@ -2123,6 +2241,11 @@
     c->L = L;
     c->obs_ptr.assign(obs_ptr, obs_ptr + L + 1);
     c->obs_idx.assign(obs_idx, obs_idx + obs_ptr[L]);
+    c->obs_int.clear();
+    c->obs_cpos.clear();
+    c->ovl_min = 0;
+    c->ovl_pairs = 0;
+    c->ovl_saved = 0.0;
     c->d_obs_ptr.release();
     c->d_obs_idx.release();
     if (int rc = c->d_obs_ptr.alloc(c, (size_t)L + 1)) return rc;
@@ -2164,11 +2287,35 @@
     HIPCHK(c, hipSetDevice(c->device));
     free_plan(c);
     free_test(c);
+    c->ovl_min = 0;
+    if (int rc = apply_overlap(c)) return rc;
     for (int l = 0; l < L; ++l) {
         c->leaves[l].op = sh[l].op;
         c->leaves[l].src = sh[l].src;
         c->leaves[l].prefix = sh[l].prefix;
     }
+    return 0;
+}
+
+int dsmgp_plan_overlap_sharing(dsmgp_ctx* c, int64_t min_shared_rows, int32_t* n_pairs, double* flops_saved) {
+    if (!c) return DSMGP_E_ARG;
+    if (n_pairs) *n_pairs = 0;
+    if (flops_saved) *flops_saved = 0.0;
+    if (c->L == 0) return fail(c, DSMGP_E_STATE, "plan_overlap_sharing before set_leaves");
+    if (min_shared_rows < 1) return fail(c, DSMGP_E_ARG, "plan_overlap_sharing: min_shared_rows must be positive");
+    c->ovl_min = min_shared_rows;
+    if (int rc = apply_overlap(c)) return rc;
+    if (n_pairs) *n_pairs = c->ovl_pairs;
+    if (flops_saved) *flops_saved = c->ovl_saved;
+    return 0;
+}
+
+int dsmgp_get_leaf_order(dsmgp_ctx* c, int32_t leaf, int64_t* rows) {
+    if (!c || !rows) return DSMGP_E_ARG;
+    if (leaf < 0 || leaf >= c->L) return fail(c, DSMGP_E_ARG, "leaf out of range");
+    const LeafHost& lf = c->leaves[leaf];
+    const std::vector<int64_t>& tab = c->obs_int.empty() ? c->obs_idx : c->obs_int;
+    std::memcpy(rows, tab.data() + lf.obs_off, sizeof(int64_t) * (size_t)lf.n);
     return 0;
 }
 
@@ -2255,6 +2402,10 @@
         if (any_prefix) {
             if (c->dinvc_prefix.count)
                 dinv_complete_kernel<<<(int)c->dinvc_prefix.count, 256, DIAGP_LDS_BYTES, c->stream>>>(c->dinvc_prefix.p);
+            for (int k = 0; c->fwd_pre.count && k < c->solve_steps; ++k) {
+                const int n = c->fwd_pre_off[k + 1] - c->fwd_pre_off[k];
+                if (n > 0) solve_fwd_kernel<<<n, 256, 0, c->stream>>>(c->fwd_pre.p + c->fwd_pre_off[k]);
+            }
             if (int rc = run_lanes(c, phases, 1, pt, true)) return rc;
         }
         {
@@ -2388,7 +2539,7 @@
         d.var = c->arenaPV + (size_t)total + lf.pv_off;
         d.macc = c->arenaPV + 2 * (size_t)total + accOff;
         d.sacc = d.macc + accTot;
-        d.zfused = (lf.owner == l && lf.op == DSMGP_SHARE_FULL) ? 1 : 0;
+        d.zfused = (lf.owner == l && (lf.op == DSMGP_SHARE_FULL || lf.ovl)) ? 1 : 0;
         accOff += (size_t)lf.ntpad;
         d.nt = lf.nt;
         d.ntpad = lf.ntpad;
@@ -3516,6 +3667,10 @@
     if (seconds) *seconds = ms * 1e-3;
     if (mu_out) HIPCHK(c, hipMemcpy(mu_out, dmu, nobs * sizeof(double), hipMemcpyDeviceToHost));
     if (var_out) HIPCHK(c, hipMemcpy(var_out, dvar, nobs * sizeof(double), hipMemcpyDeviceToHost));
+    for (int l = 0; l < L; ++l) {
+        if (mu_out) to_caller_order(c, l, mu_out + c->obs_ptr[l]);
+        if (var_out) to_caller_order(c, l, var_out + c->obs_ptr[l]);
+    }
     if (lpd_out) HIPCHK(c, hipMemcpy(lpd_out, dlpd, (size_t)L * sizeof(double), hipMemcpyDeviceToHost));
     return 0;
 }
@@ -3986,6 +4141,7 @@
     if (alpha) {
         if (int rc = ensure_alpha(c)) return rc;
         HIPCHK(c, hipMemcpy(alpha, d.alpha, lf.n * sizeof(double), hipMemcpyDeviceToHost));
+        to_caller_order(c, leaf, alpha);
     }
     return 0;
 }
diff --git a/deepstructuredmixtures_amd/csrc/host_tree.cpp b/deepstructuredmixtures_amd/csrc/host_tree.cpp
--- a/deepstructuredmixtures_amd/csrc/host_tree.cpp
+++ b/deepstructuredmixtures_amd/csrc/host_tree.cpp
@@ -141,6 +141,113 @@
 }
 
 namespace {
+struct PairCand {
+    int64_t p;
+    int32_t i, j;
+};
+}
+
+extern "C" int dsmgp_overlap_plan(int32_t L, const int64_t* obs_ptr, const int64_t* obs_idx, const int32_t* kernel_id,
+                                  const int32_t* eligible, int64_t N, int64_t min_shared_rows, int32_t* src_out, int64_t* shared_out,
+                                  int64_t* order_out, int32_t* n_pairs, double* flops_saved) {
+    if (L < 0 || !obs_ptr || (!obs_idx && L > 0 && obs_ptr[L] > 0) || !kernel_id || N <= 0 || min_shared_rows < 1 || !src_out ||
+        !shared_out || !order_out)
+        return DSMGP_E_ARG;
+    const int64_t TBL = 128;
+    const int64_t total = L ? obs_ptr[L] : 0;
+    for (int32_t l = 0; l < L; ++l)
+        if (obs_ptr[l + 1] < obs_ptr[l]) return DSMGP_E_ARG;
+    for (int64_t e = 0; e < total; ++e)
+        if (obs_idx[e] < 0 || obs_idx[e] >= N) return DSMGP_E_ARG;
+    for (int32_t l = 0; l < L; ++l)
+        for (int64_t e = obs_ptr[l] + 1; e < obs_ptr[l + 1]; ++e)
+            if (obs_idx[e] <= obs_idx[e - 1]) return DSMGP_E_ARG;
+    for (int32_t l = 0; l < L; ++l) {
+        src_out[l] = -1;
+        shared_out[l] = 0;
+    }
+    if (total) std::memcpy(order_out, obs_idx, (size_t)total * sizeof(int64_t));
+    if (n_pairs) *n_pairs = 0;
+    if (flops_saved) *flops_saved = 0.0;
+    const int64_t pmin = std::max<int64_t>(TBL, (min_shared_rows + TBL - 1) / TBL * TBL);
+    auto n_of = [&](int32_t l) { return obs_ptr[l + 1] - obs_ptr[l]; };
+    auto role = [&](int32_t l) { return eligible ? eligible[l] : 1; };
+    std::vector<int32_t> cand;
+    for (int32_t l = 0; l < L; ++l)
+        if (role(l) != 0 && n_of(l) >= pmin) cand.push_back(l);
+    if (cand.size() < 2) return 0;
+    std::vector<int64_t> pptr((size_t)N + 1, 0);
+    for (int32_t l : cand)
+        for (int64_t e = obs_ptr[l]; e < obs_ptr[l + 1]; ++e) pptr[(size_t)obs_idx[e] + 1]++;
+    for (int64_t q = 0; q < N; ++q) pptr[(size_t)q + 1] += pptr[(size_t)q];
+    std::vector<int32_t> pleaf((size_t)pptr[(size_t)N]);
+    {
+        std::vector<int64_t> fill(pptr.begin(), pptr.end() - 1);
+        for (int32_t l : cand)
+            for (int64_t e = obs_ptr[l]; e < obs_ptr[l + 1]; ++e) pleaf[(size_t)fill[(size_t)obs_idx[e]]++] = l;
+    }
+    std::vector<PairCand> pairs;
+    {
+        std::vector<int32_t> cnt((size_t)L, 0), touched;
+        for (int32_t j : cand) {
+            touched.clear();
+            for (int64_t e = obs_ptr[j]; e < obs_ptr[j + 1]; ++e) {
+                const int64_t pt = obs_idx[e];
+                for (int64_t q = pptr[(size_t)pt + 1] - 1; q >= pptr[(size_t)pt]; --q) {
+                    const int32_t l = pleaf[(size_t)q];
+                    if (l <= j) break;
+                    if (cnt[(size_t)l]++ == 0) touched.push_back(l);
+                }
+            }
+            for (int32_t l : touched) {
+                const int64_t s = cnt[(size_t)l];
+                cnt[(size_t)l] = 0;
+                if (kernel_id[l] != kernel_id[j] || (role(l) == 2 && role(j) == 2)) continue;
+                const int64_t nsh = role(j) == 2 ? n_of(l) : (role(l) == 2 ? n_of(j) : std::min(n_of(j), n_of(l)));
+                const int64_t p = std::min(s / TBL, (nsh - 1) / TBL) * TBL;
+                if (p >= pmin) pairs.push_back(PairCand{p, j, l});
+            }
+        }
+    }
+    std::sort(pairs.begin(), pairs.end(), [](const PairCand& a, const PairCand& b) {
+        if (a.p != b.p) return a.p > b.p;
+        if (a.i != b.i) return a.i < b.i;
+        return a.j < b.j;
+    });
+    std::vector<char> taken((size_t)L, 0), mark((size_t)N, 0);
+    for (const PairCand& pc : pairs) {
+        if (taken[(size_t)pc.i] || taken[(size_t)pc.j]) continue;
+        taken[(size_t)pc.i] = taken[(size_t)pc.j] = 1;
+        int32_t s = (n_of(pc.j) > n_of(pc.i)) ? pc.j : pc.i;
+        if (role(pc.i) == 2) s = pc.i;
+        if (role(pc.j) == 2) s = pc.j;
+        const int32_t t = s == pc.i ? pc.j : pc.i;
+        src_out[t] = s;
+        shared_out[s] = shared_out[t] = pc.p;
+        for (int64_t e = obs_ptr[s]; e < obs_ptr[s + 1]; ++e) mark[(size_t)obs_idx[e]] = 1;
+        int64_t got = 0;
+        for (int64_t e = obs_ptr[t]; e < obs_ptr[t + 1]; ++e) {
+            char& m = mark[(size_t)obs_idx[e]];
+            if (m == 1 && got < pc.p) {
+                m = 2;
+                ++got;
+            }
+        }
+        for (int32_t l : {s, t}) {
+            int64_t head = obs_ptr[l], tail = obs_ptr[l] + pc.p;
+            for (int64_t e = obs_ptr[l]; e < obs_ptr[l + 1]; ++e) {
+                const int64_t pt = obs_idx[e];
+                order_out[mark[(size_t)pt] == 2 ? head++ : tail++] = pt;
+            }
+        }
+        for (int64_t e = obs_ptr[s]; e < obs_ptr[s + 1]; ++e) mark[(size_t)obs_idx[e]] = 0;
+        if (n_pairs) ++*n_pairs;
+        if (flops_saved) *flops_saved += (double)pc.p * (double)pc.p * (double)pc.p / 3.0;
+    }
+    return 0;
+}
+
+namespace {
 #pragma clang fp contract(off)
 
 static double np_pairwise(const double* a, int64_t n) {
diff --git a/deepstructuredmixtures_amd/hipabi.py b/deepstructuredmixtures_amd/hipabi.py
--- a/deepstructuredmixtures_amd/hipabi.py
+++ b/deepstructuredmixtures_amd/hipabi.py
@@ -14,6 +14,10 @@
 OPT_DIAG_IN_UPDATE = 4
 OPT_FIT_GRAPH = 5
 OPT_LANES = 6
+OPT_OVERLAP_SHARE = 7
+OPT_OVERLAP_MAX_ROWS = 8
+OVERLAP_MAX_LEAF_ROWS = 8960
+OVERLAP_MIN_SHARED_ROWS = 1024
 SCORE_NAMES = ("mse", "sse", "mae", "sae", "nlpd")
 
 
@@ -36,6 +40,9 @@
     "dsmgp_set_train": (C.c_int, [_ctx, _dp, _dp, C.c_int64, C.c_int32]),
     "dsmgp_set_leaves": (C.c_int, [_ctx, C.c_int32, _lp, _lp, _ip, _dp]),
     "dsmgp_set_sharing": (C.c_int, [_ctx, _ip, _ip, _lp]),
+    "dsmgp_plan_overlap_sharing": (C.c_int, [_ctx, C.c_int64, _ip, _dp]),
+    "dsmgp_get_leaf_order": (C.c_int, [_ctx, C.c_int32, _lp]),
+    "dsmgp_overlap_plan": (C.c_int, [C.c_int32, _lp, _lp, _ip, _ip, C.c_int64, C.c_int64, _ip, _lp, _lp, _ip, _dp]),
     "dsmgp_set_hyper": (C.c_int, [_ctx, C.c_int32, C.c_int32, _dp, C.c_int32]),
     "dsmgp_fit": (C.c_int, [_ctx, _dp, _ip, _dp]),
     "dsmgp_set_test": (C.c_int, [_ctx, _dp, C.c_int64, C.c_int32, _lp, _lp]),
@@ -229,6 +236,18 @@
         plen, p2 = _i64(plen)
         self._chk(self.lib.dsmgp_set_sharing(self.h, p0, p1, p2))
 
+    def plan_overlap_sharing(self, min_shared_rows=OVERLAP_MIN_SHARED_ROWS):
+        n = C.c_int32(0)
+        f = C.c_double(0.0)
+        self._chk(self.lib.dsmgp_plan_overlap_sharing(self.h, int(min_shared_rows), C.byref(n), C.byref(f)))
+        self.overlap_pairs, self.overlap_flops_saved = n.value, f.value
+        return n.value, f.value
+
+    def leaf_order(self, leaf, n):
+        rows = np.empty(int(n), dtype=np.int64)
+        self._chk(self.lib.dsmgp_get_leaf_order(self.h, int(leaf), rows.ctypes.data_as(_lp)))
+        return rows
+
     def set_hyper(self, kernel_id, kind, loghyp):
         v, p = _f64(loghyp)
         self._chk(self.lib.dsmgp_set_hyper(self.h, int(kernel_id), int(kind), p, len(v)))
@@ -572,11 +591,17 @@
                         np.asarray(kernel_id, dtype=np.int32), np.asarray(mean, dtype=np.float64))
         self.L = len(obs_ptr) - 1
         self._sharing = (None, None, None)
+        self._overlap_min = None
         self._dirty = True
         self._test = None
 
     def set_sharing(self, op, src, plen):
         self._sharing = (None, None, None) if op is None else (np.asarray(op), np.asarray(src), np.asarray(plen))
+        self._overlap_min = None
+        self._dirty = True
+
+    def plan_overlap_sharing(self, min_shared_rows=OVERLAP_MIN_SHARED_ROWS):
+        self._overlap_min = int(min_shared_rows)
         self._dirty = True
 
     def set_hyper(self, kernel_id, kind, loghyp):
@@ -634,6 +659,12 @@
             else:
                 g2l = {int(g): i for i, g in enumerate(loc)}
                 s.set_sharing(op[loc], np.array([g2l.get(int(src[g]), -1) for g in loc], dtype=np.int32), plen[loc])
+        self.overlap_pairs, self.overlap_flops_saved = 0, 0.0
+        if self._overlap_min is not None:
+            for s in self.act:
+                n, f = s.plan_overlap_sharing(self._overlap_min)
+                self.overlap_pairs += n
+                self.overlap_flops_saved += f
         self._dirty = False
         self._test_dirty = self._test is not None
 
@@ -903,13 +934,19 @@
                         np.asarray(kernel_id, dtype=np.int32), np.asarray(mean, dtype=np.float64))
         self.L = len(obs_ptr) - 1
         self._sharing = (None, None, None)
+        self._overlap_min = None
         self._test = None
         self.groups = None
         self._res = None
 
     def set_sharing(self, op, src, plen):
         self._sharing = (None, None, None) if op is None else (np.asarray(op), np.asarray(src), np.asarray(plen))
+        self._overlap_min = None
         self.groups = None
+        self._res = None
+
+    def plan_overlap_sharing(self, min_shared_rows=OVERLAP_MIN_SHARED_ROWS):
+        self._overlap_min = int(min_shared_rows)
         self._res = None
 
     def set_hyper(self, kernel_id, kind, loghyp):
@@ -1005,6 +1042,7 @@
             return r
 
         t_pass = _time.perf_counter()
+        self.overlap_pairs, self.overlap_flops_saved = 0, 0.0
         for gi, loc in enumerate(self.groups):
             if self.verbose:
                 print(f"# streaming pass {self.passes + 1}: group {gi + 1}/{len(self.groups)} ({len(loc)} leaves) at "
@@ -1018,6 +1056,10 @@
                 g2l = {int(g): i for i, g in enumerate(loc)}
                 timed("set_sharing", c.set_sharing, op[loc],
                       np.array([g2l.get(int(src[g]), -1) for g in loc], dtype=np.int32), plen[loc])
+            if self._overlap_min is not None:
+                n_ov, f_ov = timed("set_sharing", c.plan_overlap_sharing, self._overlap_min)
+                self.overlap_pairs += n_ov
+                self.overlap_flops_saved += f_ov
             if self._test is not None:
                 Xt, rptr, ridx = self._test
                 tptr = np.concatenate([[0], np.cumsum(rptr[loc + 1] - rptr[loc])])
diff --git a/deepstructuredmixtures_amd/model.py b/deepstructuredmixtures_amd/model.py
--- a/deepstructuredmixtures_amd/model.py
+++ b/deepstructuredmixtures_amd/model.py
@@ -1,3 +1,4 @@
+import os
 import numpy as np
 
 try:
@@ -232,6 +233,13 @@
         else:
             self._set_decisions(None)
             self.ctx.set_sharing(None, None, None)
+        self.overlap_pairs, self.overlap_flops_saved = 0, 0.0
+        if (self.root.kind != "gp" and hasattr(self.ctx, "plan_overlap_sharing")
+                and os.environ.get("DSMGP_OVERLAP_SHARE", "1").strip() != "0"):
+            self.ctx.set_option(hipabi.OPT_OVERLAP_MAX_ROWS, hipabi.OVERLAP_MAX_LEAF_ROWS)
+            self.ctx.plan_overlap_sharing(hipabi.OVERLAP_MIN_SHARED_ROWS)
+            self.overlap_pairs = getattr(self.ctx, "overlap_pairs", 0)
+            self.overlap_flops_saved = getattr(self.ctx, "overlap_flops_saved", 0.0)
         self._uploaded = True
         self._schedule = key
         self._route_cache = None
diff --git a/include/dsmgp_hip.h b/include/dsmgp_hip.h
--- a/include/dsmgp_hip.h
+++ b/include/dsmgp_hip.h
@@ -49,6 +49,12 @@
 int dsmgp_set_sharing(dsmgp_ctx* ctx, const int32_t* op , const int32_t* src ,
                       const int64_t* prefix_len );
 
+int dsmgp_plan_overlap_sharing(dsmgp_ctx* ctx, int64_t min_shared_rows, int32_t* n_pairs, double* flops_saved);
+int dsmgp_get_leaf_order(dsmgp_ctx* ctx, int32_t leaf, int64_t* rows );
+int dsmgp_overlap_plan(int32_t L, const int64_t* obs_ptr, const int64_t* obs_idx, const int32_t* kernel_id, const int32_t* eligible,
+                       int64_t N, int64_t min_shared_rows, int32_t* src_out, int64_t* shared_out, int64_t* order_out,
+                       int32_t* n_pairs, double* flops_saved);
+
 int dsmgp_set_hyper(dsmgp_ctx* ctx, int32_t kernel_id, int32_t kind, const double* loghyp, int32_t n);
 
 int dsmgp_fit(dsmgp_ctx* ctx, double* mll_out , int32_t* info_out , double* seconds);
@@ -92,6 +98,8 @@
 #define DSMGP_OPT_DIAG_IN_UPDATE 4
 #define DSMGP_OPT_FIT_GRAPH 5
 #define DSMGP_OPT_LANES 6
+#define DSMGP_OPT_OVERLAP_SHARE 7
+#define DSMGP_OPT_OVERLAP_MAX_ROWS 8
 int dsmgp_set_option(dsmgp_ctx* ctx, int32_t option, int32_t value);
 int dsmgp_lanes(dsmgp_ctx* ctx, int32_t* lanes);
 
```

After: 0.3835, median of 6. Within noise of the previous version (-0.4%).
